# pyprob/pyprob

Hardware: NVIDIA H100
Metric: ic_train_traces_per_sec (higher is better)
Workload: dtype f32

## Files before the change

### pyprob_b200/csrc/net.cu

```cuda
#include <vector>
#include <string.h>
#include <stdlib.h>
#include <stdint.h>

#include "common.cuh"
#include "gemm_simt.cuh"
#include "heads.cuh"
#include "tc_grouped.cuh"
#include "tc_lstm.cuh"
#include "tc_cluster.cuh"
#include "tc_persist.cuh"
#include "obs_mlp.cuh"

using gemm::Problem;

struct HImg {
  float* k_hi = nullptr; float* k_lo = nullptr; float* mn_hi = nullptr; float* mn_lo = nullptr;
  int64_t kb = 0;
};

struct WImg {
  int64_t k_hi = 0, k_lo = 0, mn_hi = 0, mn_lo = 0;
  int kb = 0;
};
struct PackEntry {
  int64_t src_off;
  int rows, cols, ld, kb;
  int64_t k_hi, k_lo, mn_hi, mn_lo;
  int tile_start, pad_;
};

struct ppb_net {
  float* wimg = nullptr;
  int64_t wimg_floats = 0;
  std::vector<PackEntry> pack;
  PackEntry* d_pack = nullptr;
  int pack_tiles = 0;
  WImg w_ihE, w_hh;
  std::vector<WImg> w1, w2;
  WImg w_obs[PPB_MAX_OBS][PPB_MAX_FF_LAYERS];
  WImg w_fin[PPB_MAX_FF_LAYERS];
  int obs_tc = 0;
  uint64_t slot_hash[10] = {0, 0, 0, 0, 0, 0, 0, 0, 0, 0};
  const void* slot_dev[10] = {nullptr, nullptr, nullptr, nullptr, nullptr, nullptr, nullptr, nullptr, nullptr, nullptr};
  void* h_blob[2] = {nullptr, nullptr};
  cudaEvent_t ev_blob[2] = {nullptr, nullptr};
  size_t blob_cap = 0;
  int blob_idx = 0;
  ppb_net_desc desc;
  std::vector<ppb_addr_desc> addrs;
  std::vector<int64_t> type_off;
  ppb_addr_desc* d_addrs = nullptr;
  int64_t* d_type_off = nullptr;
  int64_t arena_floats = 0;
  int I = 0;
  int dh_pad = 4;
  int out_pad = 4;
  int fused_cell = 3;
  float* whh_il = nullptr;
  int64_t whh_il_floats = 0;
  void* d_lstm_steps = nullptr;
  size_t lstm_steps_cap = 0;
  int* d_lstm_progress = nullptr;
  int lstm_progress_cap = 0;
  int fused_cell_bwd = 1;
  void* d_bsteps = nullptr;
  size_t bsteps_cap = 0;
  cudaStream_t side[2] = {nullptr, nullptr};
  cudaEvent_t fork_ev[16] = {nullptr, nullptr, nullptr, nullptr, nullptr, nullptr, nullptr, nullptr,
                             nullptr, nullptr, nullptr, nullptr, nullptr, nullptr, nullptr, nullptr};
  int fork_next = 0;
  int single_stream = 0;
  int pack_tiles_no_hh = 0;
  int host_graph = 1;
  cudaStream_t host_stream = nullptr;
  cudaGraphExec_t host_exec = nullptr;
  uint64_t host_key = 0;
  int host_seen = 0;
  float* host_hyper_dev = nullptr;
  void* host_state_dev = nullptr;
  float host_hyper[6] = {0, 0, 0, 0, 0, 0};
  int64_t host_step_dev = -1;
  char* host_pin = nullptr;
  int64_t host_pin_cap = 0;
  Problem* h_stage[2] = {nullptr, nullptr};
  cudaEvent_t ev_stage[2] = {nullptr, nullptr};
  size_t stage_cap = 0;
  int stage_idx = 0;
};

namespace {

inline int64_t align_up(int64_t x, int64_t a) { return (x + a - 1) / a * a; }

struct Ws {
  float* obs_act[PPB_MAX_OBS][PPB_MAX_FF_LAYERS];
  float* obs_cat; float* fin_act[PPB_MAX_FF_LAYERS]; float* obs_emb;
  float* p_obs; float* emb_cat; float* p_step; float* w_smp_t; float* smp_emb;
  float* gates; float* c; float* h; float* hid; float* out_raw; float* row_lp; float* d_out;
  float* loss_acc;
  float* d_hid; float* dh; float* dh_rec; float* dc; float* d_pobs; float* d_pstep; float* d_smp; float* d_embcat;
  float* d_obs_emb; float* d_fin_act[PPB_MAX_FF_LAYERS]; float* d_obs_cat; float* d_obs_act[PPB_MAX_OBS][PPB_MAX_FF_LAYERS];
  Problem* problems;
  int64_t max_problems;
  int64_t total_bytes;
};

struct Dims {
  int B, R, T, NS, G;
};

Ws carve(const ppb_net* net, Dims d, void* base) {
  const ppb_net_desc& D = net->desc;
  Ws w;
  memset(&w, 0, sizeof(w));
  char* p = (char*)base;
  int64_t off = 0;
  auto take = [&](int64_t floats) {
    float* r = (float*)(p + off);
    off += align_up(floats * 4, 256);
    return r;
  };
  const int H = D.lstm_dim, E = D.obs_dim, S = D.sample_dim, C2 = 2 * (D.type_dim + D.addr_dim);
  for (int j = 0; j < D.num_obs; ++j)
    for (int l = 0; l + 1 < D.obs_ff[j].num_layers; ++l) w.obs_act[j][l] = take((int64_t)d.B * D.obs_ff[j].layers[l].out_dim);
  w.obs_cat = take((int64_t)d.B * E);
  for (int l = 0; l + 1 < D.obs_final.num_layers; ++l) w.fin_act[l] = take((int64_t)d.B * D.obs_final.layers[l].out_dim);
  w.obs_emb = take((int64_t)d.B * E);
  w.p_obs = take((int64_t)d.B * 4 * H);
  w.emb_cat = take((int64_t)d.NS * C2);
  w.p_step = take((int64_t)d.NS * 4 * H);
  w.w_smp_t = take((int64_t)S * 4 * H);
  w.smp_emb = take((int64_t)d.R * S);
  w.gates = take((int64_t)d.R * 4 * H);
  w.c = take((int64_t)d.R * H);
  w.h = take((int64_t)d.R * H);
  w.hid = take((int64_t)d.R * net->dh_pad);
  w.out_raw = take((int64_t)d.R * net->out_pad);
  w.row_lp = take(d.R);
  w.d_out = take((int64_t)d.R * net->out_pad);
  w.loss_acc = take(64);
  w.d_hid = take((int64_t)d.R * net->dh_pad);
  w.dh = take((int64_t)d.R * H);
  w.dh_rec = take((int64_t)d.R * H);
  w.dc = take((int64_t)d.R * H);
  w.d_pobs = take((int64_t)d.B * 4 * H);
  w.d_pstep = take((int64_t)d.NS * 4 * H);
  w.d_smp = take((int64_t)d.R * S);
  w.d_embcat = take((int64_t)d.NS * C2);
  w.d_obs_emb = take((int64_t)d.B * E);
  for (int l = 0; l + 1 < D.obs_final.num_layers; ++l) w.d_fin_act[l] = take((int64_t)d.B * D.obs_final.layers[l].out_dim);
  w.d_obs_cat = take((int64_t)d.B * E);
  for (int j = 0; j < D.num_obs; ++j)
    for (int l = 0; l + 1 < D.obs_ff[j].num_layers; ++l) w.d_obs_act[j][l] = take((int64_t)d.B * D.obs_ff[j].layers[l].out_dim);
  w.max_problems = 2 * (64 + 4LL * PPB_MAX_OBS * PPB_MAX_FF_LAYERS + 8LL * d.G + 4LL * d.T);
  w.problems = (Problem*)take(w.max_problems * (int64_t)(sizeof(Problem) / 4));
  w.total_bytes = off;
  return w;
}

inline float* dgates_ptr(const Ws& w, void* base) { return (float*)((char*)base + w.total_bytes); }
inline int64_t dgates_bytes(const ppb_net* net, Dims d) { return align_up((int64_t)d.R * 4 * net->desc.lstm_dim * 4, 256); }

struct Builder {
  std::vector<Problem> probs;
  std::vector<gemm::Phase> phases;
  void begin() { gemm::Phase ph; ph.first = (int)probs.size(); phases.push_back(ph); }
  void add(Problem p) {
    gemm::Phase& ph = phases.back();
    p.tiles_m = (p.M + gemm::BM - 1) / gemm::BM;
    p.tiles_n = (p.N + gemm::BN - 1) / gemm::BN;
    p.tile_start = ph.tiles;
    if (p.M <= 0 || p.N <= 0) return;
    ph.tiles += p.tiles_m * p.tiles_n;
    ph.count += 1;
    probs.push_back(p);
  }
};

inline Problem P0() {
  Problem p;
  memset(&p, 0, sizeof(p));
  p.alpha = 1.0f;
  return p;
}

inline Problem linear_fwd(const float* X, int64_t ldx, const float* W, int64_t ldw, const float* b, float* Y,
                          int64_t ldy, int M, int N, int K, int flags) {
  Problem p = P0();
  p.A = X; p.sam = ldx; p.sak = 1;
  p.B = W; p.sbn = ldw; p.sbk = 1;
  p.C = Y; p.ldc = ldy; p.bias = b;
  p.M = M; p.N = N; p.K = K; p.flags = flags;
  return p;
}
inline Problem linear_dx(const float* dY, int64_t lddy, const float* W, int64_t ldw, float* dX, int64_t lddx, int M,
                         int N, int K, int flags) {
  Problem p = P0();
  p.A = dY; p.sam = lddy; p.sak = 1;
  p.B = W; p.sbn = 1; p.sbk = ldw;
  p.C = dX; p.ldc = lddx;
  p.M = M; p.N = K; p.K = N; p.flags = flags;
  return p;
}
inline Problem linear_dw(const float* dY, int64_t lddy, const float* X, int64_t ldx, float* dW, int64_t ldw, int M,
                         int N, int K) {
  Problem p = P0();
  p.A = dY; p.sam = 1; p.sak = lddy;
  p.B = X; p.sbn = 1; p.sbk = ldx;
  p.C = dW; p.ldc = ldw;
  p.M = N; p.N = K; p.K = M; p.flags = gemm::kAccumulate;
  return p;
}

void add_obs_embed(Builder& bl, const ppb_net_desc& D, const float* arena, const float* obs, int B,
                   float* const (*obs_act)[PPB_MAX_FF_LAYERS], float* obs_cat, float* const* fin_act, float* obs_emb) {
  const int E = D.obs_dim;
  int max_depth = 0;
  for (int j = 0; j < D.num_obs; ++j) max_depth = D.obs_ff[j].num_layers > max_depth ? D.obs_ff[j].num_layers : max_depth;
  std::vector<int> in_off(D.num_obs), out_off(D.num_obs);
  { int ci = 0, co = 0; for (int j = 0; j < D.num_obs; ++j) { in_off[j] = ci; out_off[j] = co; ci += D.obs_ff[j].in_dim; co += D.obs_ff[j].out_dim; } }
  for (int l = 0; l < max_depth; ++l) {
    bl.begin();
    for (int j = 0; j < D.num_obs; ++j) {
      const ppb_ff_desc& ff = D.obs_ff[j];
      if (l >= ff.num_layers) continue;
      const ppb_linear_desc& L = ff.layers[l];
      const float* X = l == 0 ? obs + in_off[j] : obs_act[j][l - 1];
      int64_t ldx = l == 0 ? D.obs_in_total : ff.layers[l - 1].out_dim;
      bool last = (l == ff.num_layers - 1);
      float* Y = last ? obs_cat + out_off[j] : obs_act[j][l];
      int64_t ldy = last ? E : L.out_dim;
      bl.add(linear_fwd(X, ldx, arena + L.w_off, L.in_dim, arena + L.b_off, Y, ldy, B, L.out_dim, L.in_dim, gemm::kRelu));
    }
  }
  for (int l = 0; l < D.obs_final.num_layers; ++l) {
    bl.begin();
    const ppb_linear_desc& L = D.obs_final.layers[l];
    const float* X = l == 0 ? obs_cat : fin_act[l - 1];
    bool last = (l == D.obs_final.num_layers - 1);
    float* Y = last ? obs_emb : fin_act[l];
    bl.add(linear_fwd(X, L.in_dim, arena + L.w_off, L.in_dim, arena + L.b_off, Y, L.out_dim, B, L.out_dim, L.in_dim, gemm::kRelu));
  }
}

inline uint64_t fnv1a(const void* data, size_t n, uint64_t h = 1469598103934665603ULL) {
  const unsigned char* p = (const unsigned char*)data;
  for (size_t i = 0; i < n; ++i) { h ^= p[i]; h *= 1099511628211ULL; }
  return h;
}

int upload_cached(ppb_net* net, int slot, const void* src, size_t bytes, void* dev, cudaStream_t st) {
  if (bytes == 0) return PPB_OK;
  uint64_t h = fnv1a(src, bytes, 1469598103934665603ULL ^ (uint64_t)bytes);
  if (net->slot_hash[slot] == h && net->slot_dev[slot] == dev) return PPB_OK;
  cudaStreamCaptureStatus cap = cudaStreamCaptureStatusNone;
  cudaStreamIsCapturing(st, &cap);
  if (cap != cudaStreamCaptureStatusNone) {
    ppb_set_error("the batch structure changed inside a CUDA-graph capture: run the step once eagerly first");
    return PPB_EINVAL;
  }
  if (net->blob_cap < bytes) {
    for (int i = 0; i < 2; ++i) {
      if (net->h_blob[i]) cudaFreeHost(net->h_blob[i]);
      PPB_CUDA(cudaMallocHost(&net->h_blob[i], bytes * 2));
      if (!net->ev_blob[i]) PPB_CUDA(cudaEventCreateWithFlags(&net->ev_blob[i], cudaEventDisableTiming));
    }
    net->blob_cap = bytes * 2;
  }
  int i = net->blob_idx;
  net->blob_idx ^= 1;
  PPB_CUDA(cudaEventSynchronize(net->ev_blob[i]));
  memcpy(net->h_blob[i], src, bytes);
  PPB_CUDA(cudaMemcpyAsync(dev, net->h_blob[i], bytes, cudaMemcpyHostToDevice, st));
  PPB_CUDA(cudaEventRecord(net->ev_blob[i], st));
  net->slot_hash[slot] = h;
  net->slot_dev[slot] = dev;
  return PPB_OK;
}

int upload_and_get(ppb_net* net, const Builder& b, Problem* dev, int64_t cap, cudaStream_t st, int slot = 0) {
  size_t n = b.probs.size();
  if ((int64_t)n > cap) { ppb_set_error("problem list overflow (%zu > %lld)", n, (long long)cap); return PPB_ENOMEM; }
  return upload_cached(net, slot, b.probs.data(), n * sizeof(Problem), dev, st);
}

int stream_after(ppb_net* net, cudaStream_t from, cudaStream_t to) {
  if (from == to) return PPB_OK;
  cudaEvent_t& ev = net->fork_ev[net->fork_next];
  net->fork_next = (net->fork_next + 1) & 15;
  if (!ev) PPB_CUDA(cudaEventCreateWithFlags(&ev, cudaEventDisableTiming));
  PPB_CUDA(cudaEventRecord(ev, from));
  PPB_CUDA(cudaStreamWaitEvent(to, ev, 0));
  return PPB_OK;
}
int side_stream(ppb_net* net, int k, cudaStream_t main_st, cudaStream_t* out) {
  if (net->single_stream) { *out = main_st; return PPB_OK; }
  if (!net->side[k]) PPB_CUDA(cudaStreamCreateWithFlags(&net->side[k], cudaStreamNonBlocking));
  *out = net->side[k];
  return PPB_OK;
}

struct Prof {
  bool on = false;
  std::vector<std::pair<cudaEvent_t, cudaEvent_t>> spans;
  double flops = 0.0;
  int64_t launches = 0;
} g_prof;

int run_phase(const gemm::Phase& ph, const Problem* dev, cudaStream_t st, const Builder* bl_for_prof = nullptr) {
  if (ph.count == 0) return PPB_OK;
  int grid = ph.tiles < 8 * PPB_NUM_SMS ? ph.tiles : 8 * PPB_NUM_SMS;
  cudaEvent_t e0 = nullptr, e1 = nullptr;
  const bool prof = g_prof.on && bl_for_prof;
  if (prof) {
    PPB_CUDA(cudaEventCreate(&e0));
    PPB_CUDA(cudaEventCreate(&e1));
    PPB_CUDA(cudaEventRecord(e0, st));
  }
  gemm::k_grouped<<<grid, gemm::kThreads, 0, st>>>(dev + ph.first, ph.count, ph.tiles);
  PPB_LAUNCH_CHECK();
  if (prof) {
    PPB_CUDA(cudaEventRecord(e1, st));
    g_prof.spans.push_back({e0, e1});
    g_prof.launches += 1;
    for (int i = 0; i < ph.count; ++i) {
      const Problem& p = bl_for_prof->probs[ph.first + i];
      g_prof.flops += 2.0 * p.M * p.N * p.K;
    }
  }
  return PPB_OK;
}

__global__ void k_step_embed(const float* __restrict__ arena, const ppb_addr_desc* __restrict__ addrs,
                             const int64_t* __restrict__ type_off, const int* __restrict__ step_addr,
                             const int* __restrict__ step_prev, int n_steps, int td, int ad,
                             float* __restrict__ emb_cat) {
  int C2 = 2 * (td + ad);
  for (int64_t e = (int64_t)blockIdx.x * blockDim.x + threadIdx.x; e < (int64_t)n_steps * C2;
       e += (int64_t)gridDim.x * blockDim.x) {
    int st = (int)(e / C2), j = (int)(e % C2);
    int which = j < (td + ad) ? step_prev[st] : step_addr[st];
    int jj = j < (td + ad) ? j : j - (td + ad);
    float v = 0.0f;
    if (which >= 0) {
      const ppb_addr_desc& a = addrs[which];
      v = jj < td ? arena[type_off[a.type_id] + jj] : arena[a.addr_emb_off + (jj - td)];
    }
    emb_cat[e] = v;
  }
}

__global__ void k_wsmp_transpose(const float* __restrict__ w_ih, int I, int E, int S, int H4,
                                 float* __restrict__ w_smp_t) {
  for (int e = blockIdx.x * blockDim.x + threadIdx.x; e < S * H4; e += gridDim.x * blockDim.x) {
    int j = e / H4, col = e % H4;
    w_smp_t[e] = w_ih[(int64_t)col * I + E + j];
  }
}

__global__ void k_smp_embed(const float* __restrict__ arena, const ppb_addr_desc* __restrict__ addrs,
                            const int* __restrict__ row_step, const int* __restrict__ step_prev,
                            const int* __restrict__ row_prev, const float* __restrict__ values, int R, int S,
                            float* __restrict__ smp_emb) {
  for (int64_t e = (int64_t)blockIdx.x * blockDim.x + threadIdx.x; e < (int64_t)R * S;
       e += (int64_t)gridDim.x * blockDim.x) {
    int row = (int)(e / S), j = (int)(e % S);
    int pa = step_prev[row_step[row]];
    float v = 0.0f;
    if (pa >= 0) {
      const ppb_addr_desc& a = addrs[pa];
      float x = values[row_prev[row]];
      const float* W = arena + a.smp_w_off + (int64_t)j * a.smp_in;
      float pre = arena[a.smp_b_off + j];
      if (a.family == PPB_FAMILY_CATEGORICAL) {
        int c = (int)x;
        if (c >= 0 && c < a.smp_in) pre += W[c];
      } else {
        pre += W[0] * x;
      }
      v = fmaxf(pre, 0.0f);
    }
    smp_emb[e] = v;
  }
}

__global__ void __launch_bounds__(256) k_cell_fwd(float* __restrict__ gates, const float* __restrict__ p_obs,
                                                   const float* __restrict__ p_step, const float* __restrict__ w_smp_t,
                                                   const float* __restrict__ smp_emb, const int* __restrict__ row_step,
                                                   const int* __restrict__ row_prev, const int* __restrict__ row_trace,
                                                   float* __restrict__ c, float* __restrict__ h, HImg himg, int row0,
                                                   int n_rows, int H, int S, int t) {
  ppb_pdl_trigger();
  ppb_pdl_wait();
  int64_t total = (int64_t)n_rows * H;
  for (int64_t e = (int64_t)blockIdx.x * blockDim.x + threadIdx.x; e < total; e += (int64_t)gridDim.x * blockDim.x) {
    int i = (int)(e / H), j = (int)(e % H);
    int row = row0 + i;
    int st = row_step[row];
    int tr = row_trace[row];
    if (tr < 0) {
      gates[(int64_t)row * 4 * H + j] = 0.f; gates[(int64_t)row * 4 * H + H + j] = 0.f;
      gates[(int64_t)row * 4 * H + 2 * H + j] = 0.f; gates[(int64_t)row * 4 * H + 3 * H + j] = 0.f;
      c[(int64_t)row * H + j] = 0.f; h[(int64_t)row * H + j] = 0.f;
      if (himg.k_hi) tcg::img_store(himg.k_hi, himg.k_lo, himg.mn_hi, himg.mn_lo, row, j, himg.kb, 0.0f);
      continue;
    }
    float pre[4];
#pragma unroll
    for (int g = 0; g < 4; ++g) {
      int col = g * H + j;
      float v = p_obs[(int64_t)tr * 4 * H + col] + p_step[(int64_t)st * 4 * H + col];
      if (t > 0) {
        v += gates[(int64_t)row * 4 * H + col];
        for (int s = 0; s < S; ++s) v = fmaf(smp_emb[(int64_t)row * S + s], w_smp_t[(int64_t)s * 4 * H + col], v);
      }
      pre[g] = v;
    }
    float ig = ppb_cell_sigmoid(pre[0]);
    float fg = ppb_cell_sigmoid(pre[1]);
    float gg = ppb_cell_tanh(pre[2]);
    float og = ppb_cell_sigmoid(pre[3]);
    float cp = (t > 0) ? c[(int64_t)row_prev[row] * H + j] : 0.0f;
    float cn = fg * cp + ig * gg;
    float hn = og * ppb_cell_tanh(cn);
    gates[(int64_t)row * 4 * H + j] = ig;
    gates[(int64_t)row * 4 * H + H + j] = fg;
    gates[(int64_t)row * 4 * H + 2 * H + j] = gg;
    gates[(int64_t)row * 4 * H + 3 * H + j] = og;
    c[(int64_t)row * H + j] = cn;
    h[(int64_t)row * H + j] = hn;
    if (himg.k_hi) tcg::img_store(himg.k_hi, himg.k_lo, himg.mn_hi, himg.mn_lo, row, j, himg.kb, hn);
  }
}

struct NllArgs {
  const ppb_addr_desc* addrs;
  const int* row_step; const int* step_addr;
  const float* values; const float* prior0; const float* prior1;
  const int* row_trace;
  int K; float inv_batch;
  float* row_lp; float* d_out; int out_pad;
  HImg dimg;
};
__device__ __forceinline__ void nll_row(const NllArgs& A, const float* x, int row, int lane, float& local, int& bad) {
  const ppb_addr_desc* addrs = A.addrs;
  const int* row_step = A.row_step; const int* step_addr = A.step_addr;
  const float* values = A.values; const float* prior0 = A.prior0; const float* prior1 = A.prior1;
  const int* row_trace = A.row_trace;
  const int K = A.K, out_pad = A.out_pad;
  const float inv_batch = A.inv_batch;
  float* row_lp = A.row_lp; float* d_out = A.d_out;
// ... 1592 lines not shown
```

### pyprob_b200/csrc/net_tc.inc

```
extern unsigned long long* g_trace;
extern int g_trace_launch;

namespace {

inline int64_t img_floats(int64_t rows, int64_t cols) {
  return ((rows + 127) / 128) * ((cols + 31) / 32) * tc::kTileFloats;
}

__global__ void __launch_bounds__(256) k_pack_table(const float* __restrict__ arena, const PackEntry* __restrict__ tab,
                                                     int n_entries, float* __restrict__ wimg) {
  int tile = blockIdx.x;
  int lo = 0, hi = n_entries - 1;
  while (lo < hi) {
    int mid = (lo + hi + 1) >> 1;
    if (tab[mid].tile_start <= tile) lo = mid; else hi = mid - 1;
  }
  const PackEntry e = tab[lo];
  const int rt = tile - e.tile_start;
  const float* src = arena + e.src_off;
  for (int q = threadIdx.x + blockIdx.y * blockDim.x; q < 128 * e.kb * 8; q += blockDim.x * gridDim.y) {
    int c16 = q & 7, t = q >> 3;
    int cb = t % e.kb, r = t / e.kb;
    int row = rt * 128 + r, k0 = cb * 32 + c16 * 4;
    float h[4], l[4];
// ... 116 lines not shown
  net->w1.clear();
  net->w2.clear();
  for (auto& a : net->addrs) {
    net->w1.push_back(add(a.w1_off, a.head_hidden, H, H));
    net->w2.push_back(add(a.w2_off, a.head_out, a.head_hidden, a.head_hidden));
  }
  net->obs_tc = obs_tc_ok(D) ? 1 : 0;
  if (net->obs_tc) {
    for (int j = 0; j < D.num_obs; ++j)
      for (int l = 1; l < D.obs_ff[j].num_layers; ++l) {
        const ppb_linear_desc& L = D.obs_ff[j].layers[l];
        net->w_obs[j][l] = add(L.w_off, L.out_dim, L.in_dim, L.in_dim);
      }
    for (int l = 0; l < D.obs_final.num_layers; ++l) {
      const ppb_linear_desc& L = D.obs_final.layers[l];
      net->w_fin[l] = add(L.w_off, L.out_dim, L.in_dim, L.in_dim);
    }
  }
  net->pack_tiles_no_hh = tiles;
  net->w_hh = add(D.w_hh_off, 4 * H, H, H);
  net->pack_tiles = tiles;
  if (net->wimg) cudaFree(net->wimg);
  if (net->d_pack) cudaFree(net->d_pack);
  net->wimg_floats = off;
  PPB_CUDA(cudaMalloc((void**)&net->wimg, off * sizeof(float)));
  PPB_CUDA(cudaMalloc((void**)&net->d_pack, net->pack.size() * sizeof(PackEntry)));
  PPB_CUDA(cudaMemcpy(net->d_pack, net->pack.data(), net->pack.size() * sizeof(PackEntry), cudaMemcpyHostToDevice));
  if (net->fused_cell) {
    if (net->whh_il) cudaFree(net->whh_il);
    net->whh_il_floats = img_floats(4 * H, H);
    PPB_CUDA(cudaMalloc((void**)&net->whh_il, 2 * net->whh_il_floats * sizeof(float)));
  }
  return PPB_OK;
}

struct LstmPhase { int first = 0, count = 0, tiles = 0; };

template <bool X3>
int launch_lstm_seq(int tiles, const tcl::Seq* dev, int n, cudaStream_t st) {
  static bool attr_set = false;
  if (!attr_set) {
    PPB_CUDA(cudaFuncSetAttribute(tcl::k_lstm_seq<X3>, cudaFuncAttributeMaxDynamicSharedMemorySize, (int)tcl::smem_bytes()));
    attr_set = true;
  }
  tcl::k_lstm_seq<X3><<<tiles, tcg::kThreads, tcl::smem_bytes(), st>>>(dev, n);
  return PPB_OK;
}

template <bool X3>
int launch_lstm_step(const LstmPhase& ph, const tcl::Step* dev, cudaStream_t st) {
  static bool attr_set = false;
  if (!attr_set) {
    PPB_CUDA(cudaFuncSetAttribute(tcl::k_lstm_step<X3>, cudaFuncAttributeMaxDynamicSharedMemorySize, (int)tcl::smem_bytes()));
    attr_set = true;
  }
  tcl::k_lstm_step<X3><<<ph.tiles, tcg::kThreads, tcl::smem_bytes(), st>>>(dev + ph.first, ph.count);
  return PPB_OK;
}

struct TcWs {
  HImg obs_emb, h, hid, d_out, d_hid, dgates, dpobs;
  HImg a_img[PPB_MAX_OBS][PPB_MAX_FF_LAYERS], cat_img, fin_img[PPB_MAX_FF_LAYERS];
  HImg g_act[PPB_MAX_OBS][PPB_MAX_FF_LAYERS], g_cat, g_fin[PPB_MAX_FF_LAYERS], g_emb;
  char* obs_img_begin; int64_t obs_img_bytes;
  tcg::Problem* probs;
  int* ints;
  int64_t max_probs, max_ints;
  int64_t total_bytes;
};

TcWs carve_tc(const ppb_net* net, Dims d, void* base) {
  const ppb_net_desc& D = net->desc;
  TcWs w;
  char* p = (char*)base;
  int64_t off = 0;
  auto take = [&](int64_t floats) { float* r = (float*)(p + off); off += align_up(floats * 4, 1024); return r; };
  auto img = [&](int64_t rows, int64_t cols) {
    HImg im;
    int64_t n = img_floats(rows, cols);
    im.kb = (cols + 31) / 32;
    im.k_hi = take(n); im.k_lo = take(n); im.mn_hi = take(n); im.mn_lo = take(n);
    return im;
  };
  const int H = D.lstm_dim;
  w.obs_emb = img(d.B, D.obs_dim);
  w.h = img(d.R, H);
  w.hid = img(d.R, net->dh_pad);
  w.d_out = img(d.R, net->out_pad);
  w.d_hid = img(d.R, net->dh_pad);
  w.dgates = img(d.R, 4 * H);
  w.dpobs = img(d.B, 4 * H);
  w.obs_img_begin = p + off;
  if (net->obs_tc) {
    for (int j = 0; j < D.num_obs; ++j)
      for (int l = 0; l + 1 < D.obs_ff[j].num_layers; ++l) {
        w.a_img[j][l] = img(d.B, D.obs_ff[j].layers[l].out_dim);
        w.g_act[j][l] = img(d.B, D.obs_ff[j].layers[l].out_dim);
      }
    w.cat_img = img(d.B, D.obs_dim);
    w.g_cat = img(d.B, D.obs_dim);
    for (int l = 0; l + 1 < D.obs_final.num_layers; ++l) {
      w.fin_img[l] = img(d.B, D.obs_final.layers[l].out_dim);
      w.g_fin[l] = img(d.B, D.obs_final.layers[l].out_dim);
    }
    w.g_emb = img(d.B, D.obs_dim);
  }
  w.obs_img_bytes = (p + off) - w.obs_img_begin;
  w.max_probs = 2 * (16 + 6LL * d.NS + 4LL * d.G + 4LL * (PPB_MAX_OBS * PPB_MAX_FF_LAYERS + PPB_MAX_FF_LAYERS));
  w.probs = (tcg::Problem*)take(w.max_probs * (int64_t)(sizeof(tcg::Problem) / 4));
  w.max_ints = 64 + 4LL * (d.R / 32 + d.NS);
  w.ints = (int*)take(w.max_ints);
  w.total_bytes = off;
  return w;
}

inline int64_t simt_region_bytes(const ppb_net* net, Dims d) {
  return align_up(carve(net, d, nullptr).total_bytes + dgates_bytes(net, d), 1024);
}

struct TcBuilder {
  std::vector<tcg::Problem> probs;
  std::vector<gemm::Phase> phases;
  std::vector<int> ints;
  void begin() { gemm::Phase ph; ph.first = (int)probs.size(); phases.push_back(ph); }
  void add(tcg::Problem p) {
    gemm::Phase& ph = phases.back();
    if (p.M <= 0 || p.N <= 0 || p.K <= 0) return;
    p.tiles_m = (p.M + 127) / 128;
    p.tiles_n = (p.N + 127) / 128;
    p.tile_start = ph.tiles;
    if (p.k_splits < 1) p.k_splits = 1;
    ph.tiles += p.tiles_m * p.tiles_n * p.k_splits;
    ph.count += 1;
    probs.push_back(p);
  }
};

inline tcg::Operand op_k(const float* hi, const float* lo, int kb, int row0, int col0) {
  tcg::Operand o; o.hi = hi; o.lo = lo; o.k_rows = nullptr; o.kb = kb; o.mn = 0; o.row0 = row0; o.col0 = col0; return o;
}
inline tcg::Operand op_mn(const float* hi, const float* lo, int kb, int row0, int col0, const int* k_rows = nullptr) {
  tcg::Operand o; o.hi = hi; o.lo = lo; o.k_rows = k_rows; o.kb = kb; o.mn = 1; o.row0 = row0; o.col0 = col0; return o;
}
inline tcg::Problem TP0() { tcg::Problem p; memset(&p, 0, sizeof(p)); return p; }
inline tcg::Operand wk(const ppb_net* net, const WImg& w) { return op_k(net->wimg + w.k_hi, net->wimg + w.k_lo, w.kb, 0, 0); }
inline tcg::Operand wmn(const ppb_net* net, const WImg& w) { return op_mn(net->wimg + w.mn_hi, net->wimg + w.mn_lo, w.kb, 0, 0); }

inline bool tc_persistent_on() {
  const char* e = getenv("PPB_PERSISTENT");
  return !(e && e[0] == '0');
}

template <bool X3, int EPI>
int launch_tc(const gemm::Phase& ph, const tcg::Problem* dev, cudaStream_t st, unsigned long long* tr) {
  static bool attr_set = false;
  if (!attr_set) {
    PPB_CUDA(cudaFuncSetAttribute(tcg::k_grouped<X3, EPI>, cudaFuncAttributeMaxDynamicSharedMemorySize, (int)tcg::smem_bytes()));
    attr_set = true;
  }
  if (tc_persistent_on() && ph.tiles > PPB_NUM_SMS && tr == nullptr) {
    static bool attr_p = false;
    if (!attr_p) {
      PPB_CUDA(cudaFuncSetAttribute(tcp::k_grouped_persistent<X3, EPI>, cudaFuncAttributeMaxDynamicSharedMemorySize,
                                    (int)tcp::smem_bytes()));
      attr_p = true;
    }
    PPB_CUDA(ppb_launch(tcp::k_grouped_persistent<X3, EPI>, dim3(PPB_NUM_SMS), dim3(tcg::kThreads), tcp::smem_bytes(), st, 1, 0,
                        dev + ph.first, ph.count, ph.tiles));
    return PPB_OK;
  }
  PPB_CUDA(ppb_launch(tcg::k_grouped<X3, EPI>, dim3((unsigned)ph.tiles), dim3(tcg::kThreads), tcg::smem_bytes(), st, 1, 0,
                      dev + ph.first, ph.count, tr));
  return PPB_OK;
}

int run_tc_phase(const gemm::Phase& ph, const tcg::Problem* dev, int precision, cudaStream_t st, int epi,
                 const TcBuilder* bl_for_prof = nullptr) {
  if (ph.count == 0) return PPB_OK;
  cudaEvent_t e0 = nullptr, e1 = nullptr;
  const bool prof = g_prof.on && bl_for_prof;
  if (prof) {
    PPB_CUDA(cudaEventCreate(&e0));
    PPB_CUDA(cudaEventCreate(&e1));
    PPB_CUDA(cudaEventRecord(e0, st));
  }
  unsigned long long* tr = nullptr;
  if (g_trace && g_trace_launch < 256) { tr = g_trace + 16 * g_trace_launch; ++g_trace_launch; }
  int rc2 = PPB_OK;
  const bool x3 = precision == PPB_PREC_TF32X3;
  if (epi == 0) rc2 = x3 ? launch_tc<true, 0>(ph, dev, st, tr) : launch_tc<false, 0>(ph, dev, st, tr);
  else if (epi == 1) rc2 = x3 ? launch_tc<true, 1>(ph, dev, st, tr) : launch_tc<false, 1>(ph, dev, st, tr);
  else rc2 = x3 ? launch_tc<true, 2>(ph, dev, st, tr) : launch_tc<false, 2>(ph, dev, st, tr);
  if (rc2) return rc2;
  PPB_LAUNCH_CHECK();
  if (prof) {
    PPB_CUDA(cudaEventRecord(e1, st));
    g_prof.spans.push_back({e0, e1});
    g_prof.launches += 1;
    for (int i = 0; i < ph.count; ++i) {
      const tcg::Problem& p = bl_for_prof->probs[ph.first + i];
      g_prof.flops += 2.0 * p.M * p.N * p.K;
    }
  }
  return PPB_OK;
}

inline int pick_cluster(int tiles, int min_kc, bool spread_epilogue = false) {
  static const bool off = [] { const char* e = getenv("PPB_NO_CLUSTER"); return e && e[0] == '1'; }();
  if (off) return 1;
  int cs = 1;
  while (cs < 8 && tiles * cs * 2 <= PPB_NUM_SMS && (spread_epilogue || min_kc / (cs * 2) >= 2)) cs *= 2;
  return cs;
}

template <bool X3, int CS, int EPI>
int launch_cluster_tc(const gemm::Phase& ph, const tcg::Problem* dev, cudaStream_t st) {
  static bool attr_set = false;
  if (!attr_set) {
    PPB_CUDA(cudaFuncSetAttribute(tcc::k_cluster<X3, CS, EPI>, cudaFuncAttributeMaxDynamicSharedMemorySize, (int)tcc::smem_bytes()));
    attr_set = true;
  }
  unsigned long long* tr = nullptr;
  if (g_trace && g_trace_launch < 256) { tr = g_trace + 16 * g_trace_launch; ++g_trace_launch; }
  PPB_CUDA(tcc::launch_cluster(tcc::k_cluster<X3, CS, EPI>, ph.tiles * CS, CS, tcc::smem_bytes(), st, dev + ph.first, ph.count, tr));
  return PPB_OK;
}
template <bool X3, int EPI>
int launch_cluster_cs(int cs, const gemm::Phase& ph, const tcg::Problem* dev, cudaStream_t st) {
  if (cs == 2) return launch_cluster_tc<X3, 2, EPI>(ph, dev, st);
  if (cs == 4) return launch_cluster_tc<X3, 4, EPI>(ph, dev, st);
  return launch_cluster_tc<X3, 8, EPI>(ph, dev, st);
}

int run_tc_phase_auto(const gemm::Phase& ph, const tcg::Problem* dev, int precision, cudaStream_t st, int epi,
                      const TcBuilder& tb, bool profile = false) {
  if (ph.count == 0) return PPB_OK;
  int min_kc = 1 << 30;
  for (int i = 0; i < ph.count; ++i) {
    const tcg::Problem& p = tb.probs[ph.first + i];
    if (p.k_splits > 1) return run_tc_phase(ph, dev, precision, st, epi, profile ? &tb : nullptr);
    int kc = (p.K + 31) / 32;
    min_kc = kc < min_kc ? kc : min_kc;
  }
  static const bool spread = [] { const char* e = getenv("PPB_SPREAD_EPILOGUE"); return !(e && e[0] == '0'); }();
  const int cs = pick_cluster(ph.tiles, min_kc, epi == 2 && spread);
  if (cs == 1 || (epi != 0 && epi != 2)) return run_tc_phase(ph, dev, precision, st, epi, profile ? &tb : nullptr);
  cudaEvent_t e0 = nullptr, e1 = nullptr;
  const bool prof = g_prof.on && profile;
  if (prof) {
    PPB_CUDA(cudaEventCreate(&e0));
    PPB_CUDA(cudaEventCreate(&e1));
    PPB_CUDA(cudaEventRecord(e0, st));
  }
  const bool x3 = precision == PPB_PREC_TF32X3;
  int rc2;
  if (epi == 0) rc2 = x3 ? launch_cluster_cs<true, 0>(cs, ph, dev, st) : launch_cluster_cs<false, 0>(cs, ph, dev, st);
  else rc2 = x3 ? launch_cluster_cs<true, 2>(cs, ph, dev, st) : launch_cluster_cs<false, 2>(cs, ph, dev, st);
  if (rc2) return rc2;
  PPB_LAUNCH_CHECK();
  if (prof) {
    PPB_CUDA(cudaEventRecord(e1, st));
    g_prof.spans.push_back({e0, e1});
    g_prof.launches += 1;
    for (int i = 0; i < ph.count; ++i) {
      const tcg::Problem& p = tb.probs[ph.first + i];
      g_prof.flops += 2.0 * p.M * p.N * p.K;
    }
  }
  return PPB_OK;
}

template <bool X3, int CS, int SMAX>
int launch_lstm_cluster_s(const LstmPhase& ph, const tcl::Step* dev, cudaStream_t st) {
  static bool attr_set = false;
  if (!attr_set) {
    PPB_CUDA(cudaFuncSetAttribute(tcc::k_lstm_cluster<X3, CS, SMAX>, cudaFuncAttributeMaxDynamicSharedMemorySize,
                                  (int)tcc::smem_bytes()));
    attr_set = true;
  }
  unsigned long long* tr = nullptr;
  if (g_trace && g_trace_launch < 256) { tr = g_trace + 16 * g_trace_launch; ++g_trace_launch; }
  PPB_CUDA(tcc::launch_cluster(tcc::k_lstm_cluster<X3, CS, SMAX>, ph.tiles * CS, CS, tcc::smem_bytes(), st, dev + ph.first,
                               ph.count, tr));
  return PPB_OK;
}
template <bool X3, int CS>
int launch_lstm_cluster(const LstmPhase& ph, const tcl::Step* dev, int S, cudaStream_t st) {
  return S <= 4 ? launch_lstm_cluster_s<X3, CS, 4>(ph, dev, st) : launch_lstm_cluster_s<X3, CS, 8>(ph, dev, st);
}

template <bool X3, int CS>
int launch_lstm_bwd_cluster(const LstmPhase& ph, const tcc::BStep* dev, cudaStream_t st) {
  static bool attr_set = false;
  if (!attr_set) {
    PPB_CUDA(cudaFuncSetAttribute(tcc::k_lstm_bwd_cluster<X3, CS>, cudaFuncAttributeMaxDynamicSharedMemorySize, (int)tcc::smem_bytes()));
    attr_set = true;
  }
  PPB_CUDA(tcc::launch_cluster(tcc::k_lstm_bwd_cluster<X3, CS>, ph.tiles * CS, CS, tcc::smem_bytes(), st, dev + ph.first, ph.count));
  return PPB_OK;
}

inline int pad128(int n) { return (n + 127) / 128 * 128; }

inline obsmlp::Net obs_net_of(const ppb_net_desc& D) {
  obsmlp::Net n;
  n.num_obs = D.num_obs; n.obs_in_total = D.obs_in_total; n.E = D.obs_dim;
  for (int j = 0; j < PPB_MAX_OBS; ++j) n.obs_ff[j] = D.obs_ff[j];
  n.obs_final = D.obs_final;
  return n;
}
inline bool obs_fused_ok(const ppb_net_desc& D, int B) {
  constexpr int kFuseMaxWidth = obsmlp::W2;
  if (D.obs_dim > kFuseMaxWidth) return false;
  for (int j = 0; j < D.num_obs; ++j)
    for (int l = 0; l < D.obs_ff[j].num_layers; ++l)
      if (D.obs_ff[j].layers[l].in_dim > kFuseMaxWidth || D.obs_ff[j].layers[l].out_dim > kFuseMaxWidth) return false;
  for (int l = 0; l < D.obs_final.num_layers; ++l)
    if (D.obs_final.layers[l].in_dim > kFuseMaxWidth || D.obs_final.layers[l].out_dim > kFuseMaxWidth) return false;
  (void)B;
  return obsmlp::smem_bytes2(obs_net_of(D)) <= 200 * 1024;
}
inline obsmlp::Bufs obs_bufs_of(const Ws& w) {
  obsmlp::Bufs b;
  for (int j = 0; j < PPB_MAX_OBS; ++j)
    for (int l = 0; l < PPB_MAX_FF_LAYERS; ++l) b.obs_act[j][l] = w.obs_act[j][l];
  b.obs_cat = w.obs_cat;
  for (int l = 0; l < PPB_MAX_FF_LAYERS; ++l) b.fin_act[l] = w.fin_act[l];
  b.obs_emb = w.obs_emb;
  return b;
}
inline obsmlp::DBufs obs_dbufs_of(const Ws& w) {
  obsmlp::DBufs b;
  for (int j = 0; j < PPB_MAX_OBS; ++j)
    for (int l = 0; l < PPB_MAX_FF_LAYERS; ++l) b.d_obs_act[j][l] = w.d_obs_act[j][l];
  b.d_obs_cat = w.d_obs_cat;
  for (int l = 0; l < PPB_MAX_FF_LAYERS; ++l) b.d_fin_act[l] = w.d_fin_act[l];
  b.d_obs_emb = w.d_obs_emb;
  return b;
}
inline int obs_traces_per_cta(int B) {
  int t = (B + PPB_NUM_SMS - 1) / PPB_NUM_SMS;
  t = (t + obsmlp::kWarps - 1) / obsmlp::kWarps * obsmlp::kWarps;
  return t < obsmlp::kWarps ? obsmlp::kWarps : t;
}
int obs_fused_fwd(const ppb_net_desc& D, const float* arena, const float* obs, int B, const Ws& w, cudaStream_t st,
                  const HImg* emb_img = nullptr) {
  static bool attr = false;
  if (!attr) {
    PPB_CUDA(cudaFuncSetAttribute(obsmlp::k_fwd2, cudaFuncAttributeMaxDynamicSharedMemorySize, 200 * 1024));
    PPB_CUDA(cudaFuncSetAttribute(obsmlp::k_bwd2_dx, cudaFuncAttributeMaxDynamicSharedMemorySize, 200 * 1024));
    attr = true;
  }
  const obsmlp::Net n = obs_net_of(D);
  const int tpc = obs_traces_per_cta(B);
  obsmlp::Bufs bufs = obs_bufs_of(w);
  if (emb_img) {
    bufs.emb_k_hi = emb_img->k_hi; bufs.emb_k_lo = emb_img->k_lo; bufs.emb_mn_hi = emb_img->mn_hi; bufs.emb_mn_lo = emb_img->mn_lo;
    bufs.emb_kb = emb_img->kb;
  }
  obsmlp::k_fwd2<<<(B + tpc - 1) / tpc, obsmlp::kWarps * 32, obsmlp::smem_bytes2(n), st>>>(n, arena, obs, B, tpc, bufs);
  PPB_LAUNCH_CHECK();
  return PPB_OK;
}
int obs_fused_bwd(const ppb_net_desc& D, const float* arena, float* grad, const float* obs, int B, const Ws& w,
                  cudaStream_t st) {
  const obsmlp::Net n = obs_net_of(D);
  const int tpc = obs_traces_per_cta(B);
  PPB_CUDA(ppb_launch(obsmlp::k_bwd2_dx, dim3((B + tpc - 1) / tpc), dim3(obsmlp::kWarps * 32), obsmlp::smem_bytes2(n), st, 2,
                      0, n, arena, B, tpc, obs_bufs_of(w), obs_dbufs_of(w)));
  PPB_LAUNCH_CHECK();
  obsmlp::DwTable tab;
  memset(&tab, 0, sizeof(tab));
  int total = 0;
  auto add = [&](const float* dy, int ldy, const float* x, int ldx, const ppb_linear_desc& L) {
    obsmlp::DwLayer& e = tab.layer[tab.n_layers++];
    e.dy = dy; e.ldy = ldy; e.x = x; e.ldx = ldx; e.out_dim = L.out_dim; e.in_dim = L.in_dim;
    e.w_off = L.w_off; e.b_off = L.b_off; e.start = total;
    total += L.out_dim * L.in_dim + L.out_dim;
  };
  const int E = D.obs_dim;
  for (int l = 0; l < D.obs_final.num_layers; ++l) {
    const ppb_linear_desc& L = D.obs_final.layers[l];
    const bool last = l == D.obs_final.num_layers - 1;
    add(last ? w.d_obs_emb : w.d_fin_act[l], L.out_dim, l == 0 ? w.obs_cat : w.fin_act[l - 1], L.in_dim, L);
  }
  int in_off = 0, out_off = 0;
  for (int j = 0; j < D.num_obs; ++j) {
    const ppb_ff_desc& ff = D.obs_ff[j];
    for (int l = 0; l < ff.num_layers; ++l) {
      const ppb_linear_desc& L = ff.layers[l];
      const bool last = l == ff.num_layers - 1;
      const float* dy = last ? w.d_obs_cat + out_off : w.d_obs_act[j][l];
      const float* x = l == 0 ? obs + in_off : w.obs_act[j][l - 1];
      add(dy, last ? E : L.out_dim, x, l == 0 ? D.obs_in_total : ff.layers[l - 1].out_dim, L);
    }
    in_off += ff.in_dim;
    out_off += ff.out_dim;
  }
  tab.total = total;
  const int b_chunk = 512;
  PPB_CUDA(ppb_launch(obsmlp::k_dw, dim3((total + 31) / 32, (B + b_chunk - 1) / b_chunk), dim3(256), 0, st, 2, 0, tab, B,
                      b_chunk, grad));
  PPB_LAUNCH_CHECK();
  return PPB_OK;
}

inline int pick_splits(int M, int N, int K, int phase_tiles = 0) {
  int tiles = ((M + 127) / 128) * ((N + 127) / 128), kc = (K + 31) / 32;
  if (phase_tiles > tiles) tiles = phase_tiles;
  int s = PPB_NUM_SMS / tiles;
  if (s > kc / 2) s = kc / 2;
  return s < 1 ? 1 : s;
}

__global__ void __launch_bounds__(256) k_head_bias_grad(const float* __restrict__ d_out, int out_pad,
                                                         const float* __restrict__ d_hid, int dh_pad,
                                                         const int* __restrict__ head_rows, const int* __restrict__ group_start,
                                                         const int* __restrict__ group_addr,
                                                         const ppb_addr_desc* __restrict__ addrs, float* __restrict__ grad) {
  __shared__ float part[8][33];
  const int g = blockIdx.y;
  const ppb_addr_desc a = addrs[group_addr[g]];
  const int hid_blocks = (dh_pad + 31) / 32;
  const bool is_hid = (int)blockIdx.x < hid_blocks;
  const int lane = threadIdx.x & 31, slice = threadIdx.x >> 5;
  const int n = (is_hid ? blockIdx.x : blockIdx.x - hid_blocks) * 32 + lane;
  const int width = is_hid ? a.head_hidden : a.head_out;
  const float* src = is_hid ? d_hid : d_out;
  const int ld = is_hid ? dh_pad : out_pad;
  const int s0 = group_start[g], cnt = group_start[g + 1] - s0;
  float s = 0.0f;
  if (n < width)
    for (int m = slice; m < cnt; m += 8) s += src[(int64_t)head_rows[s0 + m] * ld + n];
  part[slice][lane] = s;
  __syncthreads();
  if (slice == 0 && n < width) {
    float t = 0.0f;
#pragma unroll
    for (int k = 0; k < 8; ++k) t += part[k][lane];
    if (t != 0.0f) atomicAdd(grad + (is_hid ? a.b1_off : a.b2_off) + n, t);
  }
}

__global__ void __launch_bounds__(256) k_pstep_fwd(const float* __restrict__ emb_cat, const float* __restrict__ w_ih,
                                                    const float* __restrict__ b_ih, const float* __restrict__ b_hh,
                                                    int NS, int H4, int I, int off, int C2, float* __restrict__ p_step) {
  int warp = (blockIdx.x * blockDim.x + threadIdx.x) >> 5, lane = threadIdx.x & 31;
  int nw = (gridDim.x * blockDim.x) >> 5;
  for (int o = warp; o < NS * H4; o += nw) {
    int st = o / H4, col = o % H4;
    float s = 0.0f;
    for (int j = lane; j < C2; j += 32) s = fmaf(emb_cat[(int64_t)st * C2 + j], w_ih[(int64_t)col * I + off + j], s);
    s = ppb_warp_sum(s);
    if (lane == 0) p_step[o] = s + b_ih[col] + b_hh[col];
  }
}
__global__ void __launch_bounds__(256) k_pstep_dx(const float* __restrict__ d_pstep, const float* __restrict__ w_ih,
                                                   int H4, int I, int off, int C2, float* __restrict__ d_embcat) {
  __shared__ float part[8][33];
  const int st = blockIdx.y, lane = threadIdx.x & 31, slice = threadIdx.x >> 5;
  const int j = blockIdx.x * 32 + lane;
  float s = 0.0f;
  if (j < C2)
    for (int col = blockIdx.z * 8 + slice; col < H4; col += 8 * gridDim.z)
      s = fmaf(d_pstep[(int64_t)st * H4 + col], w_ih[(int64_t)col * I + off + j], s);
  part[slice][lane] = s;
  __syncthreads();
  if (slice == 0 && j < C2) {
    float t = 0.0f;
#pragma unroll
    for (int k = 0; k < 8; ++k) t += part[k][lane];
    atomicAdd(d_embcat + (int64_t)st * C2 + j, t);
  }
}
__global__ void __launch_bounds__(256) k_pstep_dw(const float* __restrict__ d_pstep, const float* __restrict__ emb_cat,
                                                   int NS, int H4, int I, int off, int C2, float* __restrict__ dw_ih) {
  for (int64_t e = (int64_t)blockIdx.x * blockDim.x + threadIdx.x; e < (int64_t)H4 * C2;
       e += (int64_t)gridDim.x * blockDim.x) {
    int col = (int)(e / C2), j = (int)(e % C2);
    float s = 0.0f;
    for (int st = 0; st < NS; ++st) s = fmaf(d_pstep[(int64_t)st * H4 + col], emb_cat[(int64_t)st * C2 + j], s);
    dw_ih[(int64_t)col * I + off + j] += s;
  }
}

int check_tc(const ppb_net* net, const ppb_batch* b) {
  PPB_CHECK_ARG(b->row_align == 128, "the tensor-core path needs a batch encoded with row_align = 128");
  PPB_CHECK_ARG(net->wimg != nullptr, "weight images not built (ppb_net_set_tables)");
  PPB_CHECK_ARG(net->desc.lstm_dim % 32 == 0, "tensor-core path: lstm_dim must be a multiple of 32");
  PPB_CHECK_ARG(b->step_addr_host && b->step_row0_host && b->step_nrows_host && b->step_t_host && b->step_prev_row0_host,
                "missing per-step host arrays");
  return PPB_OK;
}

int tc_loss_forward(ppb_net* net, const float* arena, const ppb_batch* b, void* workspace, int precision,
                    float* loss_out, int32_t* status_out, float* row_lp_out, int want_grad, cudaStream_t st) {
  int rc = check_tc(net, b);
  if (rc) return rc;
  const ppb_net_desc& D = net->desc;
  Dims d = dims_of(b);
  Ws w = carve(net, d, workspace);
  TcWs t = carve_tc(net, d, (char*)workspace + simt_region_bytes(net, d));
  const int H = D.lstm_dim, H4 = 4 * H, E = D.obs_dim, S = D.sample_dim, I = net->I;
  const int C2 = 2 * (D.type_dim + D.addr_dim);
  const int dhkb = (net->dh_pad + 31) / 32;

  Builder bl;
  const bool fused_obs = obs_fused_ok(D, d.B);
  const bool obs_tc = !fused_obs && net->obs_tc;
  std::vector<int> obs_in_off(D.num_obs), obs_out_off(D.num_obs);
  { int ci = 0, co = 0; for (int j = 0; j < D.num_obs; ++j) { obs_in_off[j] = ci; obs_out_off[j] = co; ci += D.obs_ff[j].in_dim; co += D.obs_ff[j].out_dim; } }
  if (obs_tc) {
    bl.begin();
    for (int j = 0; j < D.num_obs; ++j) {
      const ppb_linear_desc& L = D.obs_ff[j].layers[0];
      bl.add(linear_fwd(b->obs + obs_in_off[j], D.obs_in_total, arena + L.w_off, L.in_dim, arena + L.b_off, w.obs_act[j][0],
                        L.out_dim, d.B, L.out_dim, L.in_dim, gemm::kRelu));
    }
  } else if (!fused_obs) {
    add_obs_embed(bl, D, arena, b->obs, d.B, w.obs_act, w.obs_cat, w.fin_act, w.obs_emb);
  }
  const int ph_pstep = (int)bl.phases.size();
  rc = upload_and_get(net, bl, w.problems, w.max_problems / 2, st, 0);
  if (rc) return rc;

  TcBuilder tb;
  std::vector<int> ph_obs_tc;
  if (obs_tc) {
    auto set_out = [](tcg::Problem& p, const HImg& im, int col0) {
      p.o_k_hi = im.k_hi; p.o_k_lo = im.k_lo; p.o_mn_hi = im.mn_hi; p.o_mn_lo = im.mn_lo;
      p.o_kb = (int)im.kb; p.o_row0 = 0; p.o_col0 = col0;
    };
    int max_depth = 0;
    for (int j = 0; j < D.num_obs; ++j) max_depth = D.obs_ff[j].num_layers > max_depth ? D.obs_ff[j].num_layers : max_depth;
    for (int l = 1; l < max_depth; ++l) {
      ph_obs_tc.push_back((int)tb.phases.size());
      tb.begin();
      for (int j = 0; j < D.num_obs; ++j) {
        const ppb_ff_desc& ff = D.obs_ff[j];
        if (l >= ff.num_layers) continue;
        const ppb_linear_desc& L = ff.layers[l];
        const bool last = l == ff.num_layers - 1;
        tcg::Problem p = TP0();
        p.a = op_k(t.a_img[j][l - 1].k_hi, t.a_img[j][l - 1].k_lo, (int)t.a_img[j][l - 1].kb, 0, 0);
        p.b = wk(net, net->w_obs[j][l]);
        p.M = d.B; p.N = L.out_dim; p.K = L.in_dim;
        p.flags = tcg::kRelu; p.bias = arena + L.b_off;
        if (last) { set_out(p, t.cat_img, obs_out_off[j]); p.c = w.obs_cat + obs_out_off[j]; p.ldc = E; }
        else { set_out(p, t.a_img[j][l], 0); p.c = w.obs_act[j][l]; p.ldc = L.out_dim; }
        tb.add(p);
      }
    }
    for (int l = 0; l < D.obs_final.num_layers; ++l) {
      const ppb_linear_desc& L = D.obs_final.layers[l];
      const bool last = l == D.obs_final.num_layers - 1;
      const HImg& in = l == 0 ? t.cat_img : t.fin_img[l - 1];
      ph_obs_tc.push_back((int)tb.phases.size());
      tb.begin();
      tcg::Problem p = TP0();
      p.a = op_k(in.k_hi, in.k_lo, (int)in.kb, 0, 0);
      p.b = wk(net, net->w_fin[l]);
      p.M = d.B; p.N = L.out_dim; p.K = L.in_dim;
      p.flags = tcg::kRelu; p.bias = arena + L.b_off;
      if (last) { set_out(p, t.obs_emb, 0); p.c = w.obs_emb; p.ldc = L.out_dim; }
      else { set_out(p, t.fin_img[l], 0); p.c = w.fin_act[l]; p.ldc = L.out_dim; }
      tb.add(p);
    }
  }
  const int ph_pobs = (int)tb.phases.size();
  tb.begin();
  {
    tcg::Problem p = TP0();
    p.a = op_k(t.obs_emb.k_hi, t.obs_emb.k_lo, (int)t.obs_emb.kb, 0, 0);
    p.b = wk(net, net->w_ihE);
    p.M = d.B; p.N = H4; p.K = E;
    p.c = w.p_obs; p.ldc = H4;
    tb.add(p);
  }
  std::vector<int> ph_rec(d.T, -1);
  {
    int st0 = 0;
    for (int tt = 0; tt < d.T; ++tt) {
      int st1 = st0;
      while (st1 < d.NS && b->step_t_host[st1] == tt) ++st1;
      if (tt > 0) {
        ph_rec[tt] = (int)tb.phases.size();
        tb.begin();
        for (int s = st0; s < st1; ++s) {
          tcg::Problem p = TP0();
          p.a = op_k(t.h.k_hi, t.h.k_lo, (int)t.h.kb, b->step_prev_row0_host[s], 0);
          p.b = wk(net, net->w_hh);
          p.M = pad128(b->step_nrows_host[s]); p.N = H4; p.K = H;
          p.c = w.gates + (int64_t)b->step_row0_host[s] * H4; p.ldc = H4;
          tb.add(p);
        }
      }
      st0 = st1;
    }
  }
  const int ph_h1 = (int)tb.phases.size();
  tb.begin();
  for (int s = 0; s < d.NS; ++s) {
    int aid = b->step_addr_host[s];
    const ppb_addr_desc& a = net->addrs[aid];
    tcg::Problem p = TP0();
    p.a = op_k(t.h.k_hi, t.h.k_lo, (int)t.h.kb, b->step_row0_host[s], 0);
    p.b = wk(net, net->w1[aid]);
    p.M = pad128(b->step_nrows_host[s]); p.N = a.head_hidden; p.K = H;
    p.m_valid = b->step_nrows_host[s];
    p.flags = tcg::kRelu | tcg::kZeroInvalid;
    p.bias = arena + a.b1_off;
    p.o_k_hi = t.hid.k_hi; p.o_k_lo = t.hid.k_lo; p.o_mn_hi = t.hid.mn_hi; p.o_mn_lo = t.hid.mn_lo;
    p.o_kb = dhkb; p.o_row0 = b->step_row0_host[s]; p.o_col0 = 0;
    tb.add(p);
  }
  const int ph_h2 = (int)tb.phases.size();
  tb.begin();
  for (int s = 0; s < d.NS; ++s) {
    int aid = b->step_addr_host[s];
    const ppb_addr_desc& a = net->addrs[aid];
    tcg::Problem p = TP0();
    p.a = op_k(t.hid.k_hi, t.hid.k_lo, dhkb, b->step_row0_host[s], 0);
    p.b = wk(net, net->w2[aid]);
    p.M = pad128(b->step_nrows_host[s]); p.N = a.head_out; p.K = a.head_hidden;
    p.bias = arena + a.b2_off;
    p.c = w.out_raw + (int64_t)b->step_row0_host[s] * net->out_pad; p.ldc = net->out_pad;
    tb.add(p);
  }
  PPB_CHECK_ARG((int64_t)tb.probs.size() <= t.max_probs / 2, "tensor-core problem list overflow");
  rc = upload_cached(net, 2, tb.probs.data(), tb.probs.size() * sizeof(tcg::Problem), t.probs, st);
  if (rc) return rc;

  std::vector<tcl::Step> lsteps;
  std::vector<LstmPhase> lphase(d.T);
  const bool fused_cell = net->fused_cell && net->whh_il && d.T > 1;
  bool persistent = false;
  int seq_tiles = 0, seq_count = 0, seq_counters = 0;
  if (fused_cell) {
    tcl::CellIO io;
    memset(&io, 0, sizeof(io));
    io.p_obs = w.p_obs; io.p_step = w.p_step; io.smp_emb = w.smp_emb; io.w_smp_t = w.w_smp_t;
    io.row_trace = b->row_trace; io.row_step = b->row_step; io.row_prev = b->row_prev;
    io.gates = w.gates; io.c = w.c; io.h = w.h;
    io.hk_hi = t.h.k_hi; io.hk_lo = t.h.k_lo; io.hmn_hi = t.h.mn_hi; io.hmn_lo = t.h.mn_lo; io.hkb = (int)t.h.kb;
    { static const bool nb = [] { const char* e = getenv("PPB_LSTM_B_PREFETCH"); return e && e[0] == '0'; }(); io.no_b_prefetch = nb ? 1 : 0; }
    io.H = H; io.S = S;
    const tcg::Operand a_img = op_k(t.h.k_hi, t.h.k_lo, (int)t.h.kb, 0, 0);
    const tcg::Operand b_img = op_k(net->whh_il, net->whh_il + net->whh_il_floats, H / 32, 0, 0);
    std::vector<int> seg_first(d.T + 1, 0);
    {
      int st0 = 0;
      for (int tt = 0; tt < d.T; ++tt) {
        int st1 = st0;
        while (st1 < d.NS && b->step_t_host[st1] == tt) ++st1;
        seg_first[tt] = st0;
        seg_first[tt + 1] = st1;
        st0 = st1;
      }
    }
    const int n_sub1 = seg_first[2] - seg_first[1];
    std::vector<tcl::Seq> seqs;
    if (net->fused_cell == 2) {
      for (int j = 0; j < n_sub1; ++j) {
        const int s1 = seg_first[1] + j;
        tcl::Seq q;
        memset(&q, 0, sizeof(q));
        q.a = a_img; q.b = b_img;
        q.M = pad128(b->step_nrows_host[s1]);
        q.T = 1;
        for (int tt = 1; tt < d.T; ++tt)
          if (seg_first[tt + 1] - seg_first[tt] > j) q.T = tt + 1;
        q.seg_off = b->step_row0_host[s1] - b->row_off_host[1];
        q.tiles_m = q.M / 128; q.tiles_n = H / 32;
        q.tile_start = seq_tiles;
        q.prog0 = seq_counters;
        seq_tiles += q.tiles_m * q.tiles_n;
        seq_counters += q.tiles_m;
        q.io = io;
        seqs.push_back(q);
      }
      seq_count = (int)seqs.size();
      persistent = seq_count > 0 && seq_tiles <= PPB_NUM_SMS;
    }
    size_t bytes = 0;
    std::vector<char> blob;
    if (persistent) {
      const size_t seq_bytes = seqs.size() * sizeof(tcl::Seq);
      bytes = seq_bytes + (size_t)(d.T + 1) * sizeof(int);
      blob.resize(bytes);
    } else {
      for (int tt = 1; tt < d.T; ++tt) {
        lphase[tt].first = (int)lsteps.size();
        for (int s = seg_first[tt]; s < seg_first[tt + 1]; ++s) {
          tcl::Step q;
          memset(&q, 0, sizeof(q));
          q.a = a_img; q.a.row0 = b->step_prev_row0_host[s];
          q.b = b_img;
          q.M = pad128(b->step_nrows_host[s]);
          q.row0 = b->step_row0_host[s];
          q.tiles_m = q.M / 128; q.tiles_n = H / 32;
          q.tile_start = lphase[tt].tiles;
          lphase[tt].tiles += q.tiles_m * q.tiles_n;
          lphase[tt].count += 1;
          q.io = io;
          lsteps.push_back(q);
        }
      }
      bytes = lsteps.size() * sizeof(tcl::Step);
    }
    cudaStreamCaptureStatus cap = cudaStreamCaptureStatusNone;
    cudaStreamIsCapturing(st, &cap);
    if (net->lstm_steps_cap < bytes) {
      PPB_CHECK_ARG(cap == cudaStreamCaptureStatusNone, "fused LSTM step list must be built once outside a graph capture");
      if (net->d_lstm_steps) cudaFree(net->d_lstm_steps);
      PPB_CUDA(cudaMalloc(&net->d_lstm_steps, bytes * 2));
      net->lstm_steps_cap = bytes * 2;
      net->slot_hash[7] = 0;
    }
    if (persistent) {
      if (net->lstm_progress_cap < seq_counters + 1) {
        PPB_CHECK_ARG(cap == cudaStreamCaptureStatusNone, "fused LSTM counters must be allocated outside a graph capture");
        if (net->d_lstm_progress) cudaFree(net->d_lstm_progress);
        PPB_CUDA(cudaMalloc((void**)&net->d_lstm_progress, (size_t)(seq_counters + 1) * 2 * sizeof(int)));
        net->lstm_progress_cap = (seq_counters + 1) * 2;
      }
      const size_t seq_bytes = seqs.size() * sizeof(tcl::Seq);
      for (auto& q : seqs) {
        q.row_off = (const int*)((const char*)net->d_lstm_steps + seq_bytes);
        q.progress = net->d_lstm_progress;
        q.n_counters = seq_counters;
      }
      memcpy(blob.data(), seqs.data(), seq_bytes);
      memcpy(blob.data() + seq_bytes, b->row_off_host, (size_t)(d.T + 1) * sizeof(int));
      rc = upload_cached(net, 7, blob.data(), bytes, net->d_lstm_steps, st);
    } else {
      rc = upload_cached(net, 7, lsteps.data(), bytes, net->d_lstm_steps, st);
    }
    if (rc) return rc;
  }

  cudaStream_t s1, s2;
  rc = side_stream(net, 0, st, &s1); if (rc) return rc;
  rc = side_stream(net, 1, st, &s2); if (rc) return rc;
  rc = stream_after(net, st, s1); if (rc) return rc;
  rc = stream_after(net, st, s2); if (rc) return rc;
  PPB_CUDA(cudaMemsetAsync(w.loss_acc, 0, 256, s1));
  k_pack_table<<<dim3(d.T > 1 ? net->pack_tiles : net->pack_tiles_no_hh, 8), 256, 0, s2>>>(arena, net->d_pack,
                                                                                         (int)net->pack.size(), net->wimg);
  PPB_LAUNCH_CHECK();
  if (fused_cell) {
    tcl::k_pack_whh_interleaved<<<dim3(H / 32, 8), 256, 0, s2>>>(arena + D.w_hh_off, H, net->whh_il,
                                                                 net->whh_il + net->whh_il_floats);
    PPB_LAUNCH_CHECK();
  }
  k_step_embed<<<ew_grid((int64_t)d.NS * C2), 256, 0, s1>>>(arena, net->d_addrs, net->d_type_off, b->step_addr,
                                                            b->step_prev_addr, d.NS, D.type_dim, D.addr_dim, w.emb_cat);
  PPB_LAUNCH_CHECK();
  k_pstep_fwd<<<ew_grid((int64_t)d.NS * H4 * 32), 256, 0, s1>>>(w.emb_cat, arena + D.w_ih_off, arena + D.b_ih_off,
                                                                arena + D.b_hh_off, d.NS, H4, I, E + S, C2, w.p_step);
  PPB_LAUNCH_CHECK();
  if (d.T > 1) {
    k_wsmp_transpose<<<ew_grid(S * H4), 256, 0, s1>>>(arena + D.w_ih_off, I, E, S, H4, w.w_smp_t);
    PPB_LAUNCH_CHECK();
    k_smp_embed<<<ew_grid((int64_t)d.R * S), 256, 0, s1>>>(arena, net->d_addrs, b->row_step, b->step_prev_addr,
                                                           b->row_prev, b->values, d.R, S, w.smp_emb);
    PPB_LAUNCH_CHECK();
  }
  static const bool emb_fuse_on = [] { const char* e = getenv("PPB_FUSE_PACK"); return !(e && e[0] == '0'); }();
  const bool emb_packed = fused_obs && emb_fuse_on && (d.B & 127) == 0 && (E & 31) == 0;
  if (fused_obs) { rc = obs_fused_fwd(D, arena, b->obs, d.B, w, st, emb_packed ? &t.obs_emb : nullptr); if (rc) return rc; }
  if (obs_tc && (d.B & 127))
    PPB_CUDA(cudaMemsetAsync(t.obs_img_begin, 0, (size_t)t.obs_img_bytes, st));
  for (int l = 0; l < ph_pstep; ++l) { rc = run_phase(bl.phases[l], w.problems, st); if (rc) return rc; }
  if (obs_tc) {
    for (int j = 0; j < D.num_obs; ++j) {
      const int od = D.obs_ff[j].layers[0].out_dim;
      PPB_CUDA(ppb_launch(k_pack_rows, dim3(dim3((d.B + 127) / 128, 4)), dim3(256), 0, st, 1, 0, w.obs_act[j][0], d.B, od, od, t.a_img[j][0]));
      PPB_LAUNCH_CHECK();
    }
    rc = stream_after(net, s2, st); if (rc) return rc;
    for (int ph : ph_obs_tc) { rc = run_tc_phase_auto(tb.phases[ph], t.probs, precision, st, 2, tb); if (rc) return rc; }
  } else {
    if (!emb_packed) {
      PPB_CUDA(ppb_launch(k_pack_rows, dim3(dim3((d.B + 127) / 128, 4)), dim3(256), 0, st, 1, 0, w.obs_emb, d.B, E, E, t.obs_emb));
      PPB_LAUNCH_CHECK();
// ... 138 lines not shown
    const ppb_addr_desc& a = net->addrs[aid];
    tcg::Problem p = TP0();
    p.a = op_k(t.d_out.k_hi, t.d_out.k_lo, okb, b->step_row0_host[s], 0);
    p.b = wmn(net, net->w2[aid]);
    p.M = pad128(b->step_nrows_host[s]); p.N = a.head_hidden; p.K = a.head_out;
    p.flags = tcg::kMaskImg;
    p.mask_hi = t.hid.k_hi;
    p.c = w.d_hid + (int64_t)b->step_row0_host[s] * net->dh_pad; p.ldc = net->dh_pad;
    p.o_k_hi = t.d_hid.k_hi; p.o_k_lo = t.d_hid.k_lo; p.o_mn_hi = t.d_hid.mn_hi; p.o_mn_lo = t.d_hid.mn_lo;
    p.o_kb = dhkb; p.o_row0 = b->step_row0_host[s]; p.o_col0 = 0;
    tb.add(p);
  }
  const int ph_hw = (int)tb.phases.size();
  tb.begin();
  for (int s = 0; s < d.NS; ++s) {
    int aid = b->step_addr_host[s];
    const ppb_addr_desc& a = net->addrs[aid];
    tcg::Problem p = TP0();
    p.a = op_k(t.d_hid.k_hi, t.d_hid.k_lo, dhkb, b->step_row0_host[s], 0);
    p.b = wmn(net, net->w1[aid]);
    p.M = pad128(b->step_nrows_host[s]); p.N = H; p.K = a.head_hidden;
    p.c = w.dh + (int64_t)b->step_row0_host[s] * H; p.ldc = H;
    tb.add(p);
  }
  const int ph_headw = (int)tb.phases.size();
  tb.begin();
  int headw_tiles = 0;
  for (size_t aid = 0; aid < net->addrs.size(); ++aid) {
    if (chunk_off[aid] < 0) continue;
    const ppb_addr_desc& a = net->addrs[aid];
    headw_tiles += ((a.head_out + 127) / 128) * ((a.head_hidden + 127) / 128) + ((a.head_hidden + 127) / 128) * ((H + 127) / 128);
  }
  for (size_t aid = 0; aid < net->addrs.size(); ++aid) {
    if (chunk_off[aid] < 0) continue;
    const ppb_addr_desc& a = net->addrs[aid];
    const int* kr = t.ints + chunk_off[aid];
    int nch = (int)addr_chunks[aid].size();
    tcg::Problem p2 = TP0();
    p2.a = op_mn(t.d_out.mn_hi, t.d_out.mn_lo, okb, 0, 0, kr);
    p2.b = op_mn(t.hid.mn_hi, t.hid.mn_lo, dhkb, 0, 0, kr);
    p2.M = a.head_out; p2.N = a.head_hidden; p2.K = 32 * nch;
    p2.c = grad + a.w2_off; p2.ldc = a.head_hidden; p2.flags = tcg::kAccumulate;
    p2.k_splits = pick_splits(p2.M, p2.N, p2.K, headw_tiles);
    tb.add(p2);
    tcg::Problem p1 = TP0();
    p1.a = op_mn(t.d_hid.mn_hi, t.d_hid.mn_lo, dhkb, 0, 0, kr);
    p1.b = op_mn(t.h.mn_hi, t.h.mn_lo, hkb, 0, 0, kr);
    p1.M = a.head_hidden; p1.N = H; p1.K = 32 * nch;
    p1.c = grad + a.w1_off; p1.ldc = H; p1.flags = tcg::kAccumulate;
    p1.k_splits = pick_splits(p1.M, p1.N, p1.K, headw_tiles);
    tb.add(p1);
  }
  std::vector<int> ph_rec(d.T, -1);
  std::vector<char> rec_cluster(d.T, 0);
  {
    int st1 = d.NS;
    for (int tt = d.T - 1; tt >= 1; --tt) {
      int st0 = st1;
      while (st0 > 0 && b->step_t_host[st0 - 1] == tt) --st0;
      ph_rec[tt] = (int)tb.phases.size();
      tb.begin();
      for (int s = st0; s < st1; ++s) {
        tcg::Problem p = TP0();
        p.a = op_k(t.dgates.k_hi, t.dgates.k_lo, gkb, b->step_row0_host[s], 0);
        p.b = wmn(net, net->w_hh);
        p.M = pad128(b->step_nrows_host[s]); p.N = H; p.K = H4;
        p.c = w.dh_rec + (int64_t)b->step_prev_row0_host[s] * H; p.ldc = H;
        tb.add(p);
      }
      {
        gemm::Phase& ph = tb.phases.back();
        static const int dx_cluster = [] { const char* e = getenv("PPB_REC_DX_CLUSTER"); return (e && e[0] >= '1' && e[0] <= '8') ? e[0] - '0' : 0; }();
        rec_cluster[tt] = dx_cluster && pick_cluster(ph.tiles, H4 / 32) > 1;
        if (!rec_cluster[tt]) {
          int rows = 0;
          for (int i = 0; i < ph.count; ++i) rows += tb.probs[ph.first + i].M;
          const int splits = pick_splits(rows, H, H4);
          ph.tiles = 0;
          for (int i = 0; i < ph.count; ++i) {
            tcg::Problem& p = tb.probs[ph.first + i];
            p.k_splits = splits;
            p.tile_start = ph.tiles;
            ph.tiles += p.tiles_m * p.tiles_n * splits;
          }
        }
      }
      st1 = st0;
    }
  }
  std::vector<tcc::BStep> bsteps;
  std::vector<LstmPhase> bphase(d.T);
  std::vector<int> bcs(d.T, 0);
  if (net->fused_cell_bwd) {
    tcc::BwdIO io;
    memset(&io, 0, sizeof(io));
    io.gates = w.gates; io.c = w.c; io.dh = w.dh; io.dc = w.dc; io.dgates = dgates; io.d_pobs = w.d_pobs;
    io.row_prev = b->row_prev; io.row_next = b->row_next; io.row_trace = b->row_trace;
    io.gk_hi = t.dgates.k_hi; io.gk_lo = t.dgates.k_lo; io.gmn_hi = t.dgates.mn_hi; io.gmn_lo = t.dgates.mn_lo;
    io.gkb = gkb; io.H = H;
    for (int tt = d.T - 1; tt >= 1; --tt) {
      if (!rec_cluster[tt]) continue;
      const gemm::Phase& ph = tb.phases[ph_rec[tt]];
      bcs[tt] = pick_cluster(ph.tiles, H4 / 32);
      {
        static const int cap = [] { const char* e = getenv("PPB_REC_DX_CLUSTER"); return (e && e[0] >= '2' && e[0] <= '8') ? e[0] - '0' : 8; }();
        while (bcs[tt] > cap) bcs[tt] >>= 1;
      }
      bphase[tt].first = (int)bsteps.size();
      for (int i = 0; i < ph.count; ++i) {
        const tcg::Problem& p = tb.probs[ph.first + i];
        tcc::BStep q;
        memset(&q, 0, sizeof(q));
        q.a = p.a; q.b = p.b; q.M = p.M;
        q.row0 = (int)((p.c - w.dh_rec) / H);
        q.t = tt - 1;
        q.tiles_m = p.tiles_m; q.tiles_n = p.tiles_n;
        q.tile_start = bphase[tt].tiles;
        bphase[tt].tiles += q.tiles_m * q.tiles_n;
        bphase[tt].count += 1;
        q.io = io;
        bsteps.push_back(q);
      }
    }
    const size_t bytes = bsteps.size() * sizeof(tcc::BStep);
    if (bytes > 0) {
      if (net->bsteps_cap < bytes) {
        cudaStreamCaptureStatus cap = cudaStreamCaptureStatusNone;
        cudaStreamIsCapturing(st, &cap);
        PPB_CHECK_ARG(cap == cudaStreamCaptureStatusNone, "fused BPTT step list must be built once outside a graph capture");
        if (net->d_bsteps) cudaFree(net->d_bsteps);
        PPB_CUDA(cudaMalloc(&net->d_bsteps, bytes * 2));
        net->bsteps_cap = bytes * 2;
        net->slot_hash[8] = 0;
      }
      rc = upload_cached(net, 8, bsteps.data(), bytes, net->d_bsteps, st);
      if (rc) return rc;
    }
  }

  const int ph_lstm_w = (int)tb.phases.size();
  tb.begin();
  if (!hh_a.empty()) {
    tcg::Problem p = TP0();
    p.a = op_mn(t.dgates.mn_hi, t.dgates.mn_lo, gkb, 0, 0, t.ints + hh_a_off);
    p.b = op_mn(t.h.mn_hi, t.h.mn_lo, hkb, 0, 0, t.ints + hh_b_off);
    p.M = H4; p.N = H; p.K = 32 * (int)hh_a.size();
    p.c = grad + D.w_hh_off; p.ldc = H; p.flags = tcg::kAccumulate;
    p.k_splits = pick_splits(p.M, p.N, p.K);
    tb.add(p);
  }
  {
    tcg::Problem p = TP0();
    p.a = op_mn(t.dpobs.mn_hi, t.dpobs.mn_lo, gkb, 0, 0);
    p.b = op_mn(t.obs_emb.mn_hi, t.obs_emb.mn_lo, (int)t.obs_emb.kb, 0, 0);
    p.M = H4; p.N = E; p.K = pad128(d.B);
    p.c = grad + D.w_ih_off; p.ldc = I; p.flags = tcg::kAccumulate;
    p.k_splits = pick_splits(p.M, p.N, p.K);
    tb.add(p);
    tcg::Problem q = TP0();
    q.a = op_k(t.dpobs.k_hi, t.dpobs.k_lo, gkb, 0, 0);
    q.b = wmn(net, net->w_ihE);
    q.M = d.B; q.N = E; q.K = H4;
    q.c = w.d_obs_emb; q.ldc = E;
    q.k_splits = pick_splits(q.M, q.N, q.K);
    tb.add(q);
  }
  const bool fused_obs = obs_fused_ok(D, d.B);
  const bool obs_tc = !fused_obs && net->obs_tc;
  std::vector<int> ph_bobs_dx;
  int ph_bobs_dw = -1;
  std::vector<int> obs_in_off(D.num_obs), obs_out_off(D.num_obs);
  { int ci = 0, co = 0; for (int j = 0; j < D.num_obs; ++j) { obs_in_off[j] = ci; obs_out_off[j] = co; ci += D.obs_ff[j].in_dim; co += D.obs_ff[j].out_dim; } }
  int obs_max_depth = 0;
  for (int j = 0; j < D.num_obs; ++j) obs_max_depth = D.obs_ff[j].num_layers > obs_max_depth ? D.obs_ff[j].num_layers : obs_max_depth;
  if (obs_tc) {
    const int Bp = pad128(d.B);
    auto set_out = [](tcg::Problem& p, const HImg& im) {
      p.o_k_hi = im.k_hi; p.o_k_lo = im.k_lo; p.o_mn_hi = im.mn_hi; p.o_mn_lo = im.mn_lo;
      p.o_kb = (int)im.kb; p.o_row0 = 0; p.o_col0 = 0;
    };
    struct DwSpec { const HImg* gy; int gy_col0; const HImg* x; const ppb_linear_desc* L; };
    std::vector<DwSpec> dws;
    for (int l = D.obs_final.num_layers - 1; l >= 0; --l) {
      const ppb_linear_desc& L = D.obs_final.layers[l];
      const HImg& gy = (l == D.obs_final.num_layers - 1) ? t.g_emb : t.g_fin[l];
      const HImg& x = l == 0 ? t.cat_img : t.fin_img[l - 1];
      const HImg& gx = l == 0 ? t.g_cat : t.g_fin[l - 1];
      ph_bobs_dx.push_back((int)tb.phases.size());
      tb.begin();
      tcg::Problem p = TP0();
      p.a = op_k(gy.k_hi, gy.k_lo, (int)gy.kb, 0, 0);
      p.b = wmn(net, net->w_fin[l]);
      p.M = d.B; p.N = L.in_dim; p.K = L.out_dim;
      p.flags = tcg::kMaskImg; p.mask_hi = x.k_hi;
      p.c = l == 0 ? w.d_obs_cat : w.d_fin_act[l - 1]; p.ldc = L.in_dim;
      set_out(p, gx);
      tb.add(p);
      dws.push_back({&gy, 0, &x, &L});
    }
    for (int l = obs_max_depth - 1; l >= 1; --l) {
      ph_bobs_dx.push_back((int)tb.phases.size());
      tb.begin();
      for (int j = 0; j < D.num_obs; ++j) {
        const ppb_ff_desc& ff = D.obs_ff[j];
        if (l >= ff.num_layers) continue;
        const ppb_linear_desc& L = ff.layers[l];
        const bool last = l == ff.num_layers - 1;
        const HImg& gy = last ? t.g_cat : t.g_act[j][l];
        const int gy_col0 = last ? obs_out_off[j] : 0;
        const HImg& x = t.a_img[j][l - 1];
        tcg::Problem p = TP0();
        p.a = op_k(gy.k_hi, gy.k_lo, (int)gy.kb, 0, gy_col0);
        p.b = wmn(net, net->w_obs[j][l]);
        p.M = d.B; p.N = L.in_dim; p.K = L.out_dim;
        p.flags = tcg::kMaskImg; p.mask_hi = x.k_hi;
        p.c = w.d_obs_act[j][l - 1]; p.ldc = L.in_dim;
        set_out(p, t.g_act[j][l - 1]);
        tb.add(p);
        dws.push_back({&gy, gy_col0, &x, &L});
      }
    }
    ph_bobs_dw = (int)tb.phases.size();
    tb.begin();
    int dw_tiles = 0;
    for (auto& s : dws) dw_tiles += ((s.L->out_dim + 127) / 128) * ((s.L->in_dim + 127) / 128);
    for (auto& s : dws) {
      tcg::Problem p = TP0();
      p.a = op_mn(s.gy->mn_hi, s.gy->mn_lo, (int)s.gy->kb, 0, s.gy_col0);
      p.b = op_mn(s.x->mn_hi, s.x->mn_lo, (int)s.x->kb, 0, 0);
      p.M = s.L->out_dim; p.N = s.L->in_dim; p.K = Bp;
      p.c = grad + s.L->w_off; p.ldc = s.L->in_dim; p.flags = tcg::kAccumulate;
      p.k_splits = pick_splits(p.M, p.N, p.K, dw_tiles);
      tb.add(p);
    }
  }
  PPB_CHECK_ARG((int64_t)tb.probs.size() <= t.max_probs / 2, "tensor-core problem list overflow");
  tcg::Problem* tprobs = t.probs + t.max_probs / 2;
  rc = upload_cached(net, 3, tb.probs.data(), tb.probs.size() * sizeof(tcg::Problem), tprobs, st);
  if (rc) return rc;
  rc = upload_cached(net, 4, tb.ints.data(), tb.ints.size() * sizeof(int), t.ints, st);
  if (rc) return rc;

  Builder bl;
  std::vector<int> ph_fin, ph_obs;
  int ph_obs0_dw = -1;
  if (obs_tc) {
    ph_obs0_dw = (int)bl.phases.size();
    bl.begin();
    for (int j = 0; j < D.num_obs; ++j) {
      const ppb_linear_desc& L = D.obs_ff[j].layers[0];
      bl.add(linear_dw(w.d_obs_act[j][0], L.out_dim, b->obs + obs_in_off[j], D.obs_in_total, grad + L.w_off, L.in_dim, d.B,
                       L.out_dim, L.in_dim));
    }
  }
  for (int l = D.obs_final.num_layers - 1; l >= 0 && !fused_obs && !obs_tc; --l) {
    const ppb_linear_desc& L = D.obs_final.layers[l];
    const float* X = l == 0 ? w.obs_cat : w.fin_act[l - 1];
    float* dY = (l == D.obs_final.num_layers - 1) ? w.d_obs_emb : w.d_fin_act[l];
    float* dX = l == 0 ? w.d_obs_cat : w.d_fin_act[l - 1];
    ph_fin.push_back((int)bl.phases.size());
    bl.begin();
    bl.add(linear_dw(dY, L.out_dim, X, L.in_dim, grad + L.w_off, L.in_dim, d.B, L.out_dim, L.in_dim));
    Problem px = linear_dx(dY, L.out_dim, arena + L.w_off, L.in_dim, dX, L.in_dim, d.B, L.out_dim, L.in_dim, gemm::kMaskAux);
    px.aux = X; px.ld_aux = L.in_dim;
    bl.add(px);
  }
  int max_depth = 0;
  for (int j = 0; j < D.num_obs; ++j) max_depth = D.obs_ff[j].num_layers > max_depth ? D.obs_ff[j].num_layers : max_depth;
  std::vector<int> in_off(D.num_obs), out_off(D.num_obs);
  { int ci = 0, co = 0; for (int j = 0; j < D.num_obs; ++j) { in_off[j] = ci; out_off[j] = co; ci += D.obs_ff[j].in_dim; co += D.obs_ff[j].out_dim; } }
  for (int l = max_depth - 1; l >= 0 && !fused_obs && !obs_tc; --l) {
    ph_obs.push_back((int)bl.phases.size());
    bl.begin();
    for (int j = 0; j < D.num_obs; ++j) {
      const ppb_ff_desc& ff = D.obs_ff[j];
      if (l >= ff.num_layers) continue;
      const ppb_linear_desc& L = ff.layers[l];
      bool last = (l == ff.num_layers - 1);
      const float* X = l == 0 ? b->obs + in_off[j] : w.obs_act[j][l - 1];
      int64_t ldx = l == 0 ? D.obs_in_total : ff.layers[l - 1].out_dim;
      const float* dY = last ? w.d_obs_cat + out_off[j] : w.d_obs_act[j][l];
      int64_t lddy = last ? E : L.out_dim;
      bl.add(linear_dw(dY, lddy, X, ldx, grad + L.w_off, L.in_dim, d.B, L.out_dim, L.in_dim));
      if (l > 0) {
        Problem px = linear_dx(dY, lddy, arena + L.w_off, L.in_dim, w.d_obs_act[j][l - 1], ff.layers[l - 1].out_dim, d.B, L.out_dim, L.in_dim, gemm::kMaskAux);
        px.aux = w.obs_act[j][l - 1]; px.ld_aux = ff.layers[l - 1].out_dim;
        bl.add(px);
      }
    }
  }
  Problem* dprobs = w.problems + w.max_problems / 2;
  rc = upload_and_get(net, bl, dprobs, w.max_problems / 2, st, 1);
  if (rc) return rc;

  cudaStream_t s1, s2;
  rc = side_stream(net, 0, st, &s1); if (rc) return rc;
  rc = side_stream(net, 1, st, &s2); if (rc) return rc;
  {
    bool any_splitk = false;
    for (int tt = 1; tt < d.T; ++tt) any_splitk = any_splitk || !rec_cluster[tt];
    if (any_splitk && d.T > 1)
      PPB_CUDA(cudaMemsetAsync(w.dh_rec, 0, (size_t)b->row_off_host[d.T - 1] * H * sizeof(float), st));
  }
  PPB_CUDA(cudaMemsetAsync(w.d_obs_emb, 0, (size_t)d.B * E * sizeof(float), st));
  rc = run_tc_phase_auto(tb.phases[ph_dhid], tprobs, precision, st, 2, tb); if (rc) return rc;
  rc = run_tc_phase_auto(tb.phases[ph_hw], tprobs, precision, st, 0, tb); if (rc) return rc;
  static const bool fuse_pack_on = [] { const char* e = getenv("PPB_FUSE_PACK"); return !(e && e[0] == '0'); }();
  const bool dpobs_fused = fuse_pack_on && (d.B & 127) == 0 && t.dgates.k_hi != nullptr;
  bool dpobs_packed = false;
  for (int tt = d.T - 1; tt >= 0; --tt) {
    int r0 = b->row_off_host[tt], n = b->row_off_host[tt + 1] - r0;
    int done = 0;
    if (tt + 1 < d.T) {
      if (rec_cluster[tt + 1] && net->fused_cell_bwd && bcs[tt + 1] > 1) {
        const LstmPhase& bp = bphase[tt + 1];
        const tcc::BStep* dsteps = (const tcc::BStep*)net->d_bsteps;
        const bool x3 = precision == PPB_PREC_TF32X3;
        cudaEvent_t e0 = nullptr, e1 = nullptr;
        if (g_prof.on) {
          PPB_CUDA(cudaEventCreate(&e0));
          PPB_CUDA(cudaEventCreate(&e1));
          PPB_CUDA(cudaEventRecord(e0, st));
        }
        const int cs = bcs[tt + 1];
        if (cs == 2) rc = x3 ? launch_lstm_bwd_cluster<true, 2>(bp, dsteps, st) : launch_lstm_bwd_cluster<false, 2>(bp, dsteps, st);
        else if (cs == 4) rc = x3 ? launch_lstm_bwd_cluster<true, 4>(bp, dsteps, st) : launch_lstm_bwd_cluster<false, 4>(bp, dsteps, st);
        else rc = x3 ? launch_lstm_bwd_cluster<true, 8>(bp, dsteps, st) : launch_lstm_bwd_cluster<false, 8>(bp, dsteps, st);
        if (rc) return rc;
        PPB_LAUNCH_CHECK();
        if (g_prof.on) {
          PPB_CUDA(cudaEventRecord(e1, st));
          g_prof.spans.push_back({e0, e1});
          g_prof.launches += 1;
          const gemm::Phase& ph = tb.phases[ph_rec[tt + 1]];
          for (int i = 0; i < ph.count; ++i) {
            const tcg::Problem& p = tb.probs[ph.first + i];
            g_prof.flops += 2.0 * p.M * p.N * p.K;
          }
        }
        done = b->row_off_host[tt + 2] - b->row_off_host[tt + 1];
      } else if (rec_cluster[tt + 1]) {
        rc = run_tc_phase_auto(tb.phases[ph_rec[tt + 1]], tprobs, precision, st, 0, tb, true); if (rc) return rc;
      } else {
        rc = run_tc_phase(tb.phases[ph_rec[tt + 1]], tprobs, precision, st, 1, &tb); if (rc) return rc;
      }
    }
    if (n > done) {
      if (tt == 0 && done == 0 && dpobs_fused) {
        PPB_CUDA(ppb_launch(k_cell_bwd<true>, dim3(ew_grid((int64_t)n * H)), dim3(256), 0, st, 1, 0, w.gates, w.c, w.dh, w.dh_rec,
                            w.dc, dgates, w.d_pobs, b->row_prev, b->row_next, b->row_trace, t.dgates, r0, n, H, tt, t.dpobs));
        dpobs_packed = true;
      } else {
        PPB_CUDA(ppb_launch(k_cell_bwd<false>, dim3(ew_grid((int64_t)(n - done) * H)), dim3(256), 0, st, 1, 0, w.gates, w.c, w.dh,
                            w.dh_rec, w.dc, dgates, w.d_pobs, b->row_prev, b->row_next, b->row_trace, t.dgates, r0 + done,
                            n - done, H, tt, HImg()));
      }
      PPB_LAUNCH_CHECK();
    }
  }
  rc = stream_after(net, st, s1); if (rc) return rc;
  rc = run_tc_phase(tb.phases[ph_headw], tprobs, precision, s1, 1); if (rc) return rc;
  k_head_bias_grad<<<dim3((net->dh_pad + 31) / 32 + (net->out_pad + 31) / 32, d.G), 256, 0, s1>>>(
      w.d_out, net->out_pad, w.d_hid, net->dh_pad, b->head_rows, b->group_start, b->group_addr, net->d_addrs, grad);
  PPB_LAUNCH_CHECK();
  rc = stream_after(net, st, s2); if (rc) return rc;
  const bool one_pass = S <= 4 && H4 <= 2048;
  int max_rows = 0;
  for (int s = 0; s < d.NS; ++s) max_rows = b->step_nrows_host[s] > max_rows ? b->step_nrows_host[s] : max_rows;
  if (one_pass) {
    PPB_CUDA(cudaMemsetAsync(w.d_pstep, 0, (size_t)d.NS * H4 * sizeof(float), s2));
    int slab = (d.R + 2 * PPB_NUM_SMS - 1) / (2 * PPB_NUM_SMS);
    slab = slab < 4 ? 4 : (slab > kRedSlab ? kRedSlab : slab);
    const dim3 g((max_rows + slab - 1) / slab, d.NS);
    const float* wt = d.T > 1 ? w.w_smp_t : w.p_step;
    if (H4 <= 1024)
      k_dgates_reduce<4><<<g, 256, 0, s2>>>(dgates, wt, w.smp_emb, b->values, b->step_prev_addr, b->step_row0, b->step_nrows,
                                            b->row_prev, net->d_addrs, H4, S, I, E, w.d_pstep, grad, D.w_ih_off, slab);
    else
      k_dgates_reduce<8><<<g, 256, 0, s2>>>(dgates, wt, w.smp_emb, b->values, b->step_prev_addr, b->step_row0, b->step_nrows,
                                            b->row_prev, net->d_addrs, H4, S, I, E, w.d_pstep, grad, D.w_ih_off, slab);
    PPB_LAUNCH_CHECK();
  } else {
    dim3 g((H4 + 31) / 32, d.NS);
    k_step_colsum<<<g, 256, 0, s2>>>(dgates, b->step_row0, b->step_nrows, H4, w.d_pstep);
    PPB_LAUNCH_CHECK();
  }
  PPB_CUDA(cudaMemsetAsync(w.d_embcat, 0, (size_t)d.NS * C2 * sizeof(float), s2));
  k_pstep_dx<<<dim3((C2 + 31) / 32, d.NS, 16), 256, 0, s2>>>(w.d_pstep, arena + D.w_ih_off, H4, I, E + S, C2, w.d_embcat);
  PPB_LAUNCH_CHECK();
  k_pstep_dw<<<ew_grid((int64_t)H4 * C2), 256, 0, s2>>>(w.d_pstep, w.emb_cat, d.NS, H4, I, E + S, C2, grad + D.w_ih_off);
  PPB_LAUNCH_CHECK();
  k_bias_grad<<<(H4 + 255) / 256, 256, 0, s2>>>(w.d_pstep, d.NS, H4, grad + D.b_ih_off, grad + D.b_hh_off);
  PPB_LAUNCH_CHECK();
  k_embed_scatter<<<ew_grid((int64_t)d.NS * C2), 256, 0, s2>>>(w.d_embcat, net->d_addrs, net->d_type_off, b->step_addr,
                                                               b->step_prev_addr, d.NS, D.type_dim, D.addr_dim, grad);
  PPB_LAUNCH_CHECK();
  if (d.T > 1 && !one_pass) {
    const int slab = 64;
    k_smp_bwd_seg<<<dim3((max_rows + slab - 1) / slab, d.NS), 128, 0, s2>>>(dgates, w.w_smp_t, w.smp_emb, b->values,
                                                                           b->step_prev_addr, b->step_row0, b->step_nrows,
                                                                           b->row_prev, net->d_addrs, H4, S, slab, grad);
    PPB_LAUNCH_CHECK();
    int rpb = 1024;
    dim3 g((H4 + 255) / 256, (d.R + rpb - 1) / rpb);
    k_wsmp_grad<<<g, 256, 0, s2>>>(dgates, w.smp_emb, d.R, H4, S, I, E, grad + D.w_ih_off, rpb);
    PPB_LAUNCH_CHECK();
  }
  if (!dpobs_packed) {
    PPB_CUDA(ppb_launch(k_pack_rows, dim3(dim3((d.B + 127) / 128, 64)), dim3(256), 0, st, 1, 0, w.d_pobs, d.B, H4, H4, t.dpobs));
    PPB_LAUNCH_CHECK();
  }
  rc = run_tc_phase(tb.phases[ph_lstm_w], tprobs, precision, st, 1, &tb); if (rc) return rc;
  if (fused_obs) {
    rc = obs_fused_bwd(D, arena, grad, b->obs, d.B, w, st); if (rc) return rc;
    rc = stream_after(net, s1, st); if (rc) return rc;
    return stream_after(net, s2, st);
  }
  if (obs_tc) {
    PPB_CUDA(ppb_launch(k_pack_rows_masked, dim3(dim3((d.B + 127) / 128, 4)), dim3(256), 0, st, 1, 0, w.d_obs_emb, w.obs_emb, d.B, E, E, t.g_emb));
    PPB_LAUNCH_CHECK();
    for (int ph : ph_bobs_dx) { rc = run_tc_phase_auto(tb.phases[ph], tprobs, precision, st, 2, tb); if (rc) return rc; }
    rc = run_tc_phase(tb.phases[ph_bobs_dw], tprobs, precision, st, 1); if (rc) return rc;
    for (int l = 0; l < D.obs_final.num_layers; ++l) {
      const ppb_linear_desc& L = D.obs_final.layers[l];
      const float* dY = (l == D.obs_final.num_layers - 1) ? w.d_obs_emb : w.d_fin_act[l];
      k_colsum_gather<<<dim3((L.out_dim + 31) / 32, 8), 256, 0, st>>>(dY, L.out_dim, nullptr, d.B, L.out_dim, grad + L.b_off);
      PPB_LAUNCH_CHECK();
    }
    for (int j = 0; j < D.num_obs; ++j) {
      const ppb_ff_desc& ff = D.obs_ff[j];
      for (int l = 0; l < ff.num_layers; ++l) {
        const ppb_linear_desc& L = ff.layers[l];
        const bool last = l == ff.num_layers - 1;
        const float* dY = last ? w.d_obs_cat + obs_out_off[j] : w.d_obs_act[j][l];
        k_colsum_gather<<<dim3((L.out_dim + 31) / 32, 8), 256, 0, st>>>(dY, last ? E : L.out_dim, nullptr, d.B, L.out_dim,
                                                                        grad + L.b_off);
        PPB_LAUNCH_CHECK();
      }
    }
    rc = run_phase(bl.phases[ph_obs0_dw], dprobs, st); if (rc) return rc;
    rc = stream_after(net, s1, st); if (rc) return rc;
    return stream_after(net, s2, st);
  }
  k_mask_nonpos<<<ew_grid((int64_t)d.B * E), 256, 0, st>>>(w.d_obs_emb, w.obs_emb, (int64_t)d.B * E);
  PPB_LAUNCH_CHECK();
  for (size_t k = 0; k < ph_fin.size(); ++k) {
    int l = D.obs_final.num_layers - 1 - (int)k;
    const ppb_linear_desc& L = D.obs_final.layers[l];
    float* dY = (l == D.obs_final.num_layers - 1) ? w.d_obs_emb : w.d_fin_act[l];
    k_colsum_gather<<<dim3((L.out_dim + 31) / 32, 8), 256, 0, st>>>(dY, L.out_dim, nullptr, d.B, L.out_dim, grad + L.b_off);
    PPB_LAUNCH_CHECK();
    rc = run_phase(bl.phases[ph_fin[k]], dprobs, st); if (rc) return rc;
  }
  for (size_t k = 0; k < ph_obs.size(); ++k) {
    int l = max_depth - 1 - (int)k;
    for (int j = 0; j < D.num_obs; ++j) {
      const ppb_ff_desc& ff = D.obs_ff[j];
      if (l >= ff.num_layers) continue;
      const ppb_linear_desc& L = ff.layers[l];
      bool last = (l == ff.num_layers - 1);
      const float* dY = last ? w.d_obs_cat + out_off[j] : w.d_obs_act[j][l];
      int64_t lddy = last ? E : L.out_dim;
      k_colsum_gather<<<dim3((L.out_dim + 31) / 32, 8), 256, 0, st>>>(dY, lddy, nullptr, d.B, L.out_dim, grad + L.b_off);
      PPB_LAUNCH_CHECK();
    }
    rc = run_phase(bl.phases[ph_obs[k]], dprobs, st); if (rc) return rc;
  }
  rc = stream_after(net, s1, st); if (rc) return rc;
  return stream_after(net, s2, st);
}

}
```

### pyprob_b200/csrc/obs_mlp.cuh

```cuda
#pragma once
#include "common.cuh"
#include "tc.cuh"

namespace obsmlp {

constexpr int TB = 4;
constexpr int WMAX = 256;
constexpr int LD = WMAX + 1;
constexpr int NC = 64;
constexpr int kThreads = 256;

struct Bufs {
  float* obs_act[PPB_MAX_OBS][PPB_MAX_FF_LAYERS];
  float* obs_cat;
  float* fin_act[PPB_MAX_FF_LAYERS];
  float* obs_emb;
  float* emb_k_hi = nullptr; float* emb_k_lo = nullptr; float* emb_mn_hi = nullptr; float* emb_mn_lo = nullptr;
  long long emb_kb = 0;
};

struct Net {
  int num_obs, obs_in_total, E;
  ppb_ff_desc obs_ff[PPB_MAX_OBS];
  ppb_ff_desc obs_final;
};

inline size_t smem_bytes() { return (size_t)(3 * TB * LD + WMAX * (NC + 1)) * sizeof(float); }

__device__ __forceinline__ void dense_fwd(const float (*in_s)[LD], int in_dim, const float* __restrict__ W,
                                          const float* __restrict__ b, int out_dim, float (*out_s)[LD], int out_col0,
                                          float* ws, float* gout, int64_t ldg, int gcol0, int r0, int B) {
  const int tid = threadIdx.x;
  for (int n0 = 0; n0 < out_dim; n0 += NC) {
    const int nc = out_dim - n0 < NC ? out_dim - n0 : NC;
    for (int idx = tid; idx < nc * in_dim; idx += kThreads) {
      int nn = idx / in_dim, k = idx - nn * in_dim;
      ws[k * (NC + 1) + nn] = __ldg(W + (int64_t)(n0 + nn) * in_dim + k);
    }
    __syncthreads();
    for (int o = tid; o < TB * NC; o += kThreads) {
      int r = o / NC, nn = o % NC;
      if (nn < nc) {
        float acc = __ldg(b + n0 + nn);
#pragma unroll 4
        for (int k = 0; k < in_dim; ++k) acc = fmaf(in_s[r][k], ws[k * (NC + 1) + nn], acc);
        acc = fmaxf(acc, 0.0f);
        out_s[r][out_col0 + n0 + nn] = acc;
        if (r0 + r < B) gout[(int64_t)(r0 + r) * ldg + gcol0 + n0 + nn] = acc;
      }
    }
    __syncthreads();
  }
}

__global__ void __launch_bounds__(kThreads) k_fwd(Net net, const float* __restrict__ arena, const float* __restrict__ obs,
                                                   int B, Bufs bufs) {
  extern __shared__ float smem[];
  float (*cat)[LD] = reinterpret_cast<float (*)[LD]>(smem);
  float (*pa)[LD] = reinterpret_cast<float (*)[LD]>(smem + TB * LD);
  float (*pb)[LD] = reinterpret_cast<float (*)[LD]>(smem + 2 * TB * LD);
  float* ws = smem + 3 * TB * LD;
  const int r0 = blockIdx.x * TB, tid = threadIdx.x;
  int in_off = 0, out_off = 0;
  for (int j = 0; j < net.num_obs; ++j) {
    const ppb_ff_desc& ff = net.obs_ff[j];
    for (int idx = tid; idx < TB * ff.in_dim; idx += kThreads) {
      int r = idx / ff.in_dim, k = idx % ff.in_dim;
      pa[r][k] = (r0 + r < B) ? __ldg(obs + (int64_t)(r0 + r) * net.obs_in_total + in_off + k) : 0.0f;
    }
    __syncthreads();
    float (*cur)[LD] = pa;
    float (*nxt)[LD] = pb;
    for (int l = 0; l < ff.num_layers; ++l) {
      const ppb_linear_desc& L = ff.layers[l];
      const bool last = l == ff.num_layers - 1;
      if (last) dense_fwd(cur, L.in_dim, arena + L.w_off, arena + L.b_off, L.out_dim, cat, out_off, ws, bufs.obs_cat, net.E, out_off, r0, B);
      else dense_fwd(cur, L.in_dim, arena + L.w_off, arena + L.b_off, L.out_dim, nxt, 0, ws, bufs.obs_act[j][l], L.out_dim, 0, r0, B);
      float (*t)[LD] = cur; cur = nxt; nxt = t;
    }
    in_off += ff.in_dim;
    out_off += ff.out_dim;
  }
  float (*cur)[LD] = cat;
  float (*nxt)[LD] = pa;
  for (int l = 0; l < net.obs_final.num_layers; ++l) {
    const ppb_linear_desc& L = net.obs_final.layers[l];
    const bool last = l == net.obs_final.num_layers - 1;
    dense_fwd(cur, L.in_dim, arena + L.w_off, arena + L.b_off, L.out_dim, nxt, 0, ws, last ? bufs.obs_emb : bufs.fin_act[l],
              L.out_dim, 0, r0, B);
    cur = nxt;
    nxt = (nxt == pa) ? pb : pa;
  }
}

__device__ __forceinline__ void dense_bwd(const float (*dy_s)[LD], int dy_col0, int out_dim, const float* __restrict__ x,
                                          int64_t ldx, int xcol0, int in_dim, const float* __restrict__ W,
                                          float* __restrict__ dW, float* __restrict__ db, float (*x_s)[LD],
                                          float (*dx_s)[LD], bool want_dx, int r0, int B) {
  const int tid = threadIdx.x;
  for (int idx = tid; idx < TB * in_dim; idx += kThreads) {
    int r = idx / in_dim, k = idx % in_dim;
    x_s[r][k] = (r0 + r < B) ? __ldg(x + (int64_t)(r0 + r) * ldx + xcol0 + k) : 0.0f;
  }
  __syncthreads();
  for (int idx = tid; idx < out_dim * in_dim; idx += kThreads) {
    int n = idx / in_dim, k = idx - n * in_dim;
    float s = 0.0f;
#pragma unroll
    for (int r = 0; r < TB; ++r) s = fmaf(dy_s[r][dy_col0 + n], x_s[r][k], s);
    if (s != 0.0f) atomicAdd(dW + idx, s);
  }
  for (int n = tid; n < out_dim; n += kThreads) {
    float s = 0.0f;
#pragma unroll
    for (int r = 0; r < TB; ++r) s += dy_s[r][dy_col0 + n];
    if (s != 0.0f) atomicAdd(db + n, s);
  }
  if (want_dx) {
    for (int idx = tid; idx < TB * in_dim; idx += kThreads) {
      int r = idx / in_dim, k = idx - r * in_dim;
      float s = 0.0f;
      for (int n = 0; n < out_dim; ++n) s = fmaf(dy_s[r][dy_col0 + n], __ldg(W + (int64_t)n * in_dim + k), s);
      dx_s[r][k] = x_s[r][k] > 0.0f ? s : 0.0f;
    }
  }
  __syncthreads();
}

__global__ void __launch_bounds__(kThreads) k_bwd(Net net, const float* __restrict__ arena, float* __restrict__ grad,
                                                   const float* __restrict__ obs, const float* __restrict__ d_obs_emb,
                                                   int B, Bufs bufs) {
  extern __shared__ float smem[];
  float (*da)[LD] = reinterpret_cast<float (*)[LD]>(smem);
  float (*dbuf)[LD] = reinterpret_cast<float (*)[LD]>(smem + TB * LD);
  float (*xs)[LD] = reinterpret_cast<float (*)[LD]>(smem + 2 * TB * LD);
  const int r0 = blockIdx.x * TB, tid = threadIdx.x, E = net.E;
  for (int idx = tid; idx < TB * E; idx += kThreads) {
    int r = idx / E, k = idx % E;
    float g = 0.0f;
    if (r0 + r < B) {
      int64_t o = (int64_t)(r0 + r) * E + k;
      g = bufs.obs_emb[o] > 0.0f ? d_obs_emb[o] : 0.0f;
    }
    da[r][k] = g;
  }
  __syncthreads();
  float (*cur)[LD] = da;
  float (*nxt)[LD] = dbuf;
  for (int l = net.obs_final.num_layers - 1; l >= 0; --l) {
    const ppb_linear_desc& L = net.obs_final.layers[l];
    const float* x = l == 0 ? bufs.obs_cat : bufs.fin_act[l - 1];
    dense_bwd(cur, 0, L.out_dim, x, L.in_dim, 0, L.in_dim, arena + L.w_off, grad + L.w_off, grad + L.b_off, xs, nxt, true, r0, B);
    float (*t)[LD] = cur; cur = nxt; nxt = t;
  }
  float (*dcat)[LD] = cur;
  float (*tmp)[LD] = nxt;
  float (*tmp2)[LD] = reinterpret_cast<float (*)[LD]>(smem + 3 * TB * LD);
  int in_off = 0, out_off = 0;
  for (int j = 0; j < net.num_obs; ++j) {
    const ppb_ff_desc& ff = net.obs_ff[j];
    const float (*dy)[LD] = dcat;
    int dy_col0 = out_off;
    float (*o1)[LD] = tmp;
    float (*o2)[LD] = tmp2;
    for (int l = ff.num_layers - 1; l >= 0; --l) {
      const ppb_linear_desc& L = ff.layers[l];
      const float* x = l == 0 ? obs : bufs.obs_act[j][l - 1];
      int64_t ldx = l == 0 ? net.obs_in_total : ff.layers[l - 1].out_dim;
      int xcol0 = l == 0 ? in_off : 0;
      dense_bwd(dy, dy_col0, L.out_dim, x, ldx, xcol0, L.in_dim, arena + L.w_off, grad + L.w_off, grad + L.b_off, xs, o1,
                l > 0, r0, B);
      dy = o1; dy_col0 = 0;
      float (*t)[LD] = o1; o1 = o2; o2 = t;
    }
    in_off += ff.in_dim;
    out_off += ff.out_dim;
  }
}

inline size_t smem_bytes_bwd() { return (size_t)(4 * TB * LD) * sizeof(float); }

constexpr int W2 = 96;
constexpr int TPW = 1;
constexpr int kWarps = 8;

struct DBufs {
  float* d_obs_act[PPB_MAX_OBS][PPB_MAX_FF_LAYERS];
  float* d_obs_cat;
  float* d_fin_act[PPB_MAX_FF_LAYERS];
  float* d_obs_emb;
};

__host__ __device__ inline int layer_floats(const ppb_linear_desc& L) { return L.out_dim * (L.in_dim | 1) + L.out_dim; }
__host__ __device__ inline int weights_floats(const Net& net) {
  int n = 0;
  for (int j = 0; j < net.num_obs; ++j)
    for (int l = 0; l < net.obs_ff[j].num_layers; ++l) n += layer_floats(net.obs_ff[j].layers[l]);
  for (int l = 0; l < net.obs_final.num_layers; ++l) n += layer_floats(net.obs_final.layers[l]);
  return n;
}
inline size_t smem_bytes2(const Net& net) { return (size_t)(weights_floats(net) + kWarps * 3 * W2) * sizeof(float); }

__device__ __forceinline__ void cp_async4(float* smem_dst, const float* gmem_src) {
  asm volatile("cp.async.ca.shared.global [%0], [%1], 4;" ::"r"((uint32_t)__cvta_generic_to_shared(smem_dst)), "l"(gmem_src)
               : "memory");
}
__device__ __forceinline__ void cp_async_wait_all() {
  asm volatile("cp.async.commit_group;" ::: "memory");
  asm volatile("cp.async.wait_group 0;" ::: "memory");
}
__device__ __forceinline__ float* stage_layer(float* dst, const float* __restrict__ arena, const ppb_linear_desc& L) {
  const int pitch = L.in_dim | 1, nw = L.out_dim * L.in_dim;
  for (int idx = threadIdx.x; idx < nw; idx += blockDim.x) {
    int n = idx / L.in_dim, k = idx - n * L.in_dim;
    cp_async4(dst + n * pitch + k, arena + L.w_off + idx);
  }
  float* bias = dst + L.out_dim * pitch;
  for (int n = threadIdx.x; n < L.out_dim; n += blockDim.x) cp_async4(bias + n, arena + L.b_off + n);
  return bias + L.out_dim;
}

__device__ __forceinline__ void warp_dense_fwd(const float* in, int in_dim, const float* w, int out_dim, float* out,
                                               int out_col0, float* gout, int lane) {
  const int pitch = in_dim | 1;
  const float* bias = w + out_dim * pitch;
  const bool p0 = lane < out_dim, p1 = lane + 32 < out_dim, p2 = lane + 64 < out_dim;
  const float* r0 = w + (p0 ? lane : 0) * pitch;
  const float* r1 = w + (p1 ? lane + 32 : 0) * pitch;
  const float* r2 = w + (p2 ? lane + 64 : 0) * pitch;
  float a0 = p0 ? bias[lane] : 0.f, a1 = p1 ? bias[lane + 32] : 0.f, a2 = p2 ? bias[lane + 64] : 0.f;
  if (out_dim <= 32) {
#pragma unroll 4
    for (int k = 0; k < in_dim; ++k) a0 = fmaf(in[k], r0[k], a0);
  } else if (out_dim <= 64) {
#pragma unroll 4
    for (int k = 0; k < in_dim; ++k) { const float x = in[k]; a0 = fmaf(x, r0[k], a0); a1 = fmaf(x, r1[k], a1); }
  } else {
#pragma unroll 4
    for (int k = 0; k < in_dim; ++k) { const float x = in[k]; a0 = fmaf(x, r0[k], a0); a1 = fmaf(x, r1[k], a1); a2 = fmaf(x, r2[k], a2); }
  }
  a0 = fmaxf(a0, 0.f); a1 = fmaxf(a1, 0.f); a2 = fmaxf(a2, 0.f);
  if (p0) { out[out_col0 + lane] = a0; gout[lane] = a0; }
  if (p1) { out[out_col0 + lane + 32] = a1; gout[lane + 32] = a1; }
  if (p2) { out[out_col0 + lane + 64] = a2; gout[lane + 64] = a2; }
  __syncwarp();
}

__global__ void __launch_bounds__(kWarps * 32) k_fwd2(Net net, const float* __restrict__ arena,
                                                      const float* __restrict__ obs, int B, int traces_per_cta, Bufs bufs) {
  ppb_pdl_trigger();
  extern __shared__ float smem[];
  float* p = smem;
  const float* w_obs[PPB_MAX_OBS][PPB_MAX_FF_LAYERS];
  const float* w_fin[PPB_MAX_FF_LAYERS];
  for (int j = 0; j < net.num_obs; ++j)
    for (int l = 0; l < net.obs_ff[j].num_layers; ++l) { w_obs[j][l] = p; p = stage_layer(p, arena, net.obs_ff[j].layers[l]); }
  for (int l = 0; l < net.obs_final.num_layers; ++l) { w_fin[l] = p; p = stage_layer(p, arena, net.obs_final.layers[l]); }
  const int warp = threadIdx.x >> 5, lane = threadIdx.x & 31;
  float* cat = p + warp * 3 * W2;
  float* va = cat + W2;
  float* vb = va + W2;
  cp_async_wait_all();
  __syncthreads();
  const int t0 = blockIdx.x * traces_per_cta;
  for (int tr = t0 + warp; tr < t0 + traces_per_cta && tr < B; tr += kWarps) {
    int in_off = 0, out_off = 0;
    for (int j = 0; j < net.num_obs; ++j) {
      const ppb_ff_desc& ff = net.obs_ff[j];
      float* cur = va;
      float* nxt = vb;
      for (int k = lane; k < ff.in_dim; k += 32) cur[k] = __ldg(obs + (int64_t)tr * net.obs_in_total + in_off + k);
      __syncwarp();
      for (int l = 0; l < ff.num_layers; ++l) {
        const ppb_linear_desc& L = ff.layers[l];
        const bool last = l == ff.num_layers - 1;
        if (last) warp_dense_fwd(cur, L.in_dim, w_obs[j][l], L.out_dim, cat, out_off, bufs.obs_cat + (int64_t)tr * net.E + out_off, lane);
        else warp_dense_fwd(cur, L.in_dim, w_obs[j][l], L.out_dim, nxt, 0, bufs.obs_act[j][l] + (int64_t)tr * L.out_dim, lane);
        float* t = cur; cur = nxt; nxt = t;
      }
      in_off += ff.in_dim;
      out_off += ff.out_dim;
    }
    float* cur = cat;
    float* nxt = va;
    for (int l = 0; l < net.obs_final.num_layers; ++l) {
      const ppb_linear_desc& L = net.obs_final.layers[l];
      const bool last = l == net.obs_final.num_layers - 1;
      warp_dense_fwd(cur, L.in_dim, w_fin[l], L.out_dim, nxt, 0,
                     (last ? bufs.obs_emb : bufs.fin_act[l]) + (int64_t)tr * L.out_dim, lane);
      float* t = cur; cur = nxt; nxt = (t == cat) ? vb : t;
    }
    if (bufs.emb_k_hi) {
      for (int k = lane; k < net.E; k += 32) {
        float hi, lo;
        tc::split_tf32(cur[k], hi, lo);
        const int64_t ok = tc::packed_offset(tr, k, bufs.emb_kb);
        bufs.emb_k_hi[ok] = hi;
        if (bufs.emb_k_lo) bufs.emb_k_lo[ok] = lo;
        if (bufs.emb_mn_hi) {
          const int64_t om = tc::packed_offset_mn(tr, k, bufs.emb_kb);
          bufs.emb_mn_hi[om] = hi;
          if (bufs.emb_mn_lo) bufs.emb_mn_lo[om] = lo;
        }
      }
    }
    __syncwarp();
  }
}

__device__ __forceinline__ void warp_dense_dx(const float* dy, int out_dim, const float* w, int in_dim,
                                              const float* __restrict__ x, float* dx, float* gdx, int lane) {
  const int pitch = in_dim | 1;
  const bool p0 = lane < in_dim, p1 = lane + 32 < in_dim, p2 = lane + 64 < in_dim;
  const float x0 = p0 ? __ldg(x + lane) : 0.f, x1 = p1 ? __ldg(x + lane + 32) : 0.f, x2 = p2 ? __ldg(x + lane + 64) : 0.f;
  const float* c0 = w + (p0 ? lane : 0);
  const float* c1 = w + (p1 ? lane + 32 : 0);
  const float* c2 = w + (p2 ? lane + 64 : 0);
  float a0 = 0.f, a1 = 0.f, a2 = 0.f;
  if (in_dim <= 32) {
#pragma unroll 4
    for (int n = 0; n < out_dim; ++n) a0 = fmaf(dy[n], c0[n * pitch], a0);
  } else if (in_dim <= 64) {
#pragma unroll 4
    for (int n = 0; n < out_dim; ++n) { const float g = dy[n]; a0 = fmaf(g, c0[n * pitch], a0); a1 = fmaf(g, c1[n * pitch], a1); }
  } else {
#pragma unroll 4
    for (int n = 0; n < out_dim; ++n) { const float g = dy[n]; a0 = fmaf(g, c0[n * pitch], a0); a1 = fmaf(g, c1[n * pitch], a1); a2 = fmaf(g, c2[n * pitch], a2); }
  }
  if (p0) { a0 = x0 > 0.f ? a0 : 0.f; dx[lane] = a0; gdx[lane] = a0; }
  if (p1) { a1 = x1 > 0.f ? a1 : 0.f; dx[lane + 32] = a1; gdx[lane + 32] = a1; }
  if (p2) { a2 = x2 > 0.f ? a2 : 0.f; dx[lane + 64] = a2; gdx[lane + 64] = a2; }
  __syncwarp();
}

__global__ void __launch_bounds__(kWarps * 32) k_bwd2_dx(Net net, const float* __restrict__ arena, int B, int traces_per_cta,
                                                         Bufs bufs, DBufs dbufs) {
  ppb_pdl_trigger();
  ppb_pdl_wait();
  extern __shared__ float smem[];
  float* p = smem;
  const float* w_obs[PPB_MAX_OBS][PPB_MAX_FF_LAYERS];
  const float* w_fin[PPB_MAX_FF_LAYERS];
  for (int j = 0; j < net.num_obs; ++j)
    for (int l = 0; l < net.obs_ff[j].num_layers; ++l) {
      w_obs[j][l] = p;
      if (l > 0) p = stage_layer(p, arena, net.obs_ff[j].layers[l]);
    }
  for (int l = 0; l < net.obs_final.num_layers; ++l) { w_fin[l] = p; p = stage_layer(p, arena, net.obs_final.layers[l]); }
  const int warp = threadIdx.x >> 5, lane = threadIdx.x & 31, E = net.E;
  float* va = p + warp * 3 * W2;
  float* vb = va + W2;
  float* vc = vb + W2;
  cp_async_wait_all();
  __syncthreads();
  const int t0 = blockIdx.x * traces_per_cta;
  for (int tr = t0 + warp; tr < t0 + traces_per_cta && tr < B; tr += kWarps) {
    for (int k = lane; k < E; k += 32) {
      int64_t o = (int64_t)tr * E + k;
      float g = bufs.obs_emb[o] > 0.f ? dbufs.d_obs_emb[o] : 0.f;
      va[k] = g;
      dbufs.d_obs_emb[o] = g;
    }
    __syncwarp();
    float* cur = va;
    float* nxt = vb;
    for (int l = net.obs_final.num_layers - 1; l >= 0; --l) {
      const ppb_linear_desc& L = net.obs_final.layers[l];
      const float* x = (l == 0 ? bufs.obs_cat : bufs.fin_act[l - 1]) + (int64_t)tr * L.in_dim;
      float* gdx = (l == 0 ? dbufs.d_obs_cat : dbufs.d_fin_act[l - 1]) + (int64_t)tr * L.in_dim;
      warp_dense_dx(cur, L.out_dim, w_fin[l], L.in_dim, x, nxt, gdx, lane);
      float* t = cur; cur = nxt; nxt = t;
    }
    float* dcat = cur;
    float* scratch = nxt;
    int out_off = 0;
    for (int j = 0; j < net.num_obs; ++j) {
      const ppb_ff_desc& ff = net.obs_ff[j];
      const float* dy = dcat + out_off;
      float* o1 = scratch;
      float* o2 = vc;
      for (int l = ff.num_layers - 1; l >= 1; --l) {
        const ppb_linear_desc& L = ff.layers[l];
        const float* x = bufs.obs_act[j][l - 1] + (int64_t)tr * L.in_dim;
        warp_dense_dx(dy, L.out_dim, w_obs[j][l], L.in_dim, x, o1, dbufs.d_obs_act[j][l - 1] + (int64_t)tr * L.in_dim, lane);
        dy = o1;
        float* t = o1; o1 = o2; o2 = t;
      }
      out_off += ff.out_dim;
    }
    __syncwarp();
  }
}

struct DwLayer { const float* dy; const float* x; int ldy, ldx, out_dim, in_dim, start, pad_; int64_t w_off, b_off; };
struct DwTable { int n_layers, total; DwLayer layer[PPB_MAX_OBS * PPB_MAX_FF_LAYERS + PPB_MAX_FF_LAYERS]; };

__global__ void __launch_bounds__(256) k_dw(DwTable tab, int B, int b_chunk, float* __restrict__ grad) {
  ppb_pdl_trigger();
  ppb_pdl_wait();
  __shared__ float part[8][33];
  const int lane = threadIdx.x & 31, warp = threadIdx.x >> 5;
  const int idx = blockIdx.x * 32 + lane;
  float s = 0.f;
  int li = 0, e = 0, nw = 0;
  const bool live = idx < tab.total;
  if (live) {
    while (li + 1 < tab.n_layers && tab.layer[li + 1].start <= idx) ++li;
    const DwLayer& L = tab.layer[li];
    e = idx - L.start;
    nw = L.out_dim * L.in_dim;
    const int b0 = blockIdx.y * b_chunk, b1 = min(B, b0 + b_chunk);
    if (e < nw) {
      const int n = e / L.in_dim, k = e - n * L.in_dim;
      const float* dy = L.dy + n;
      const float* x = L.x + k;
#pragma unroll 8
      for (int b = b0 + warp; b < b1; b += 8) s = fmaf(__ldg(dy + (int64_t)b * L.ldy), __ldg(x + (int64_t)b * L.ldx), s);
    } else {
      const float* dy = L.dy + (e - nw);
#pragma unroll 8
      for (int b = b0 + warp; b < b1; b += 8) s += __ldg(dy + (int64_t)b * L.ldy);
    }
  }
  part[warp][lane] = s;
  __syncthreads();
  if (warp == 0 && live) {
    float t = 0.f;
#pragma unroll
    for (int w = 0; w < 8; ++w) t += part[w][lane];
    const DwLayer& L = tab.layer[li];
    if (t != 0.f) atomicAdd(grad + (e < nw ? L.w_off + e : L.b_off + (e - nw)), t);
  }
}

}
```

Baseline: 1.459 million.

## Rewrite obs MLP as plan-driven fused kernels and fuse pstep backward

Replaces the observation MLP forward and backward kernels with plan-driven versions that process tiles of traces in shared memory. The backward now computes weight gradients per CTA and reduces them across a thread-block cluster through distributed shared memory before issuing atomics, replacing the separate dx and dw kernels. It also merges the pstep dx, dw, bias and embedding-scatter kernels into one launch and adds a z-split to the head bias gradient. Workspace buffers are reordered so a single memset clears d_pstep through d_obs_emb. The aim is fewer launches and less global traffic, at the cost of larger shared-memory use and more complex indexing.

```diff
diff --git a/pyprob_b200/csrc/net.cu b/pyprob_b200/csrc/net.cu
--- a/pyprob_b200/csrc/net.cu
+++ b/pyprob_b200/csrc/net.cu
@@ -145,9 +145,9 @@
   w.dh_rec = take((int64_t)d.R * H);
   w.dc = take((int64_t)d.R * H);
   w.d_pobs = take((int64_t)d.B * 4 * H);
-  w.d_pstep = take((int64_t)d.NS * 4 * H);
   w.d_smp = take((int64_t)d.R * S);
   w.d_embcat = take((int64_t)d.NS * C2);
+  w.d_pstep = take((int64_t)d.NS * 4 * H);
   w.d_obs_emb = take((int64_t)d.B * E);
   for (int l = 0; l + 1 < D.obs_final.num_layers; ++l) w.d_fin_act[l] = take((int64_t)d.B * D.obs_final.layers[l].out_dim);
   w.d_obs_cat = take((int64_t)d.B * E);
diff --git a/pyprob_b200/csrc/net_tc.inc b/pyprob_b200/csrc/net_tc.inc
--- a/pyprob_b200/csrc/net_tc.inc
+++ b/pyprob_b200/csrc/net_tc.inc
@@ -442,12 +442,64 @@
 
 inline int pad128(int n) { return (n + 127) / 128 * 128; }
 
-inline obsmlp::Net obs_net_of(const ppb_net_desc& D) {
-  obsmlp::Net n;
-  n.num_obs = D.num_obs; n.obs_in_total = D.obs_in_total; n.E = D.obs_dim;
-  for (int j = 0; j < PPB_MAX_OBS; ++j) n.obs_ff[j] = D.obs_ff[j];
-  n.obs_final = D.obs_final;
-  return n;
+inline obsmlp::Plan obs_plan_of(const ppb_net_desc& D, const Ws* w, const float* obs) {
+  obsmlp::Plan P;
+  memset(&P, 0, sizeof(P));
+  const int E = D.obs_dim;
+  P.E = E;
+  int nf = 0;
+  auto add_layer = [&](const ppb_linear_desc& L) -> obsmlp::Layer& {
+    obsmlp::Layer& o = P.L[P.n_layers++];
+    o.in_dim = L.in_dim; o.out_dim = L.out_dim; o.w_off = L.w_off; o.b_off = L.b_off;
+    o.pitch = (L.in_dim & 3) ? L.in_dim : ((L.in_dim & 7) ? L.in_dim : L.in_dim + 4);
+    o.sw = nf;
+    nf += (L.out_dim * o.pitch + L.out_dim + 3) & ~3;
+    o.part = P.part_floats;
+    P.part_floats += L.out_dim * L.in_dim + L.out_dim;
+    return o;
+  };
+  std::vector<int> first(D.num_obs);
+  int in_off = 0;
+  for (int j = 0; j < D.num_obs; ++j) {
+    const ppb_ff_desc& ff = D.obs_ff[j];
+    first[j] = P.n_layers;
+    for (int l = 0; l < ff.num_layers; ++l) {
+      obsmlp::Layer& o = add_layer(ff.layers[l]);
+      o.xoff = P.A; P.A += o.in_dim;
+      if (l + 1 < ff.num_layers) { o.dzoff = P.Dz; P.Dz += o.out_dim; }
+      o.dxoff = l == 0 ? -1 : P.L[P.n_layers - 2].dzoff;
+      o.x = l == 0 ? obs + in_off : (w ? w->obs_act[j][l - 1] : nullptr);
+      o.ldx = l == 0 ? D.obs_in_total : ff.layers[l - 1].out_dim;
+      if (l + 1 < ff.num_layers) { o.y = w ? w->obs_act[j][l] : nullptr; o.ldy = o.out_dim; }
+    }
+    in_off += ff.in_dim;
+  }
+  const int cat = P.A, dcat = P.Dz;
+  P.A += E; P.Dz += E;
+  int out_off = 0;
+  for (int j = 0; j < D.num_obs; ++j) {
+    obsmlp::Layer& o = P.L[first[j] + D.obs_ff[j].num_layers - 1];
+    o.yoff = cat + out_off; o.dzoff = dcat + out_off;
+    o.y = w ? w->obs_cat + out_off : nullptr; o.ldy = E;
+    out_off += D.obs_ff[j].out_dim;
+  }
+  for (int j = 0; j < D.num_obs; ++j)
+    for (int l = 0; l + 1 < D.obs_ff[j].num_layers; ++l) P.L[first[j] + l].yoff = P.L[first[j] + l + 1].xoff;
+  const int nfin = D.obs_final.num_layers;
+  for (int l = 0; l < nfin; ++l) {
+    const bool last = l == nfin - 1;
+    obsmlp::Layer& o = add_layer(D.obs_final.layers[l]);
+    if (l == 0) o.xoff = cat;
+    o.yoff = P.A; P.A += o.out_dim;
+    o.dzoff = P.Dz; P.Dz += o.out_dim;
+    o.dxoff = l == 0 ? dcat : P.L[P.n_layers - 2].dzoff;
+    o.x = l == 0 ? (w ? w->obs_cat : nullptr) : (w ? w->fin_act[l - 1] : nullptr);
+    o.ldx = o.in_dim;
+    o.y = w ? (last ? w->obs_emb : w->fin_act[l]) : nullptr; o.ldy = o.out_dim;
+    if (l > 0) o.xoff = P.L[P.n_layers - 2].yoff;
+  }
+  P.w_floats = nf;
+  return P;
 }
 inline bool obs_fused_ok(const ppb_net_desc& D, int B) {
   constexpr int kFuseMaxWidth = obsmlp::W2;
@@ -458,89 +510,44 @@
   for (int l = 0; l < D.obs_final.num_layers; ++l)
     if (D.obs_final.layers[l].in_dim > kFuseMaxWidth || D.obs_final.layers[l].out_dim > kFuseMaxWidth) return false;
   (void)B;
-  return obsmlp::smem_bytes2(obs_net_of(D)) <= 200 * 1024;
-}
-inline obsmlp::Bufs obs_bufs_of(const Ws& w) {
-  obsmlp::Bufs b;
-  for (int j = 0; j < PPB_MAX_OBS; ++j)
-    for (int l = 0; l < PPB_MAX_FF_LAYERS; ++l) b.obs_act[j][l] = w.obs_act[j][l];
-  b.obs_cat = w.obs_cat;
-  for (int l = 0; l < PPB_MAX_FF_LAYERS; ++l) b.fin_act[l] = w.fin_act[l];
-  b.obs_emb = w.obs_emb;
-  return b;
-}
-inline obsmlp::DBufs obs_dbufs_of(const Ws& w) {
-  obsmlp::DBufs b;
-  for (int j = 0; j < PPB_MAX_OBS; ++j)
-    for (int l = 0; l < PPB_MAX_FF_LAYERS; ++l) b.d_obs_act[j][l] = w.d_obs_act[j][l];
-  b.d_obs_cat = w.d_obs_cat;
-  for (int l = 0; l < PPB_MAX_FF_LAYERS; ++l) b.d_fin_act[l] = w.d_fin_act[l];
-  b.d_obs_emb = w.d_obs_emb;
-  return b;
-}
-inline int obs_traces_per_cta(int B) {
-  int t = (B + PPB_NUM_SMS - 1) / PPB_NUM_SMS;
-  t = (t + obsmlp::kWarps - 1) / obsmlp::kWarps * obsmlp::kWarps;
-  return t < obsmlp::kWarps ? obsmlp::kWarps : t;
+  const obsmlp::Plan P = obs_plan_of(D, nullptr, nullptr);
+  return obsmlp::smem_fwd(P) <= obsmlp::kMaxSmem && obsmlp::smem_bwd(P) <= obsmlp::kMaxSmem;
+}
+int obs_set_smem_limits() {
+  static bool attr = false;
+  if (!attr) {
+    PPB_CUDA(cudaFuncSetAttribute(obsmlp::k_fwd, cudaFuncAttributeMaxDynamicSharedMemorySize, (int)obsmlp::kMaxSmem));
+    PPB_CUDA(cudaFuncSetAttribute(obsmlp::k_bwd, cudaFuncAttributeMaxDynamicSharedMemorySize, (int)obsmlp::kMaxSmem));
+    attr = true;
+  }
+  return PPB_OK;
 }
 int obs_fused_fwd(const ppb_net_desc& D, const float* arena, const float* obs, int B, const Ws& w, cudaStream_t st,
                   const HImg* emb_img = nullptr) {
-  static bool attr = false;
-  if (!attr) {
-    PPB_CUDA(cudaFuncSetAttribute(obsmlp::k_fwd2, cudaFuncAttributeMaxDynamicSharedMemorySize, 200 * 1024));
-    PPB_CUDA(cudaFuncSetAttribute(obsmlp::k_bwd2_dx, cudaFuncAttributeMaxDynamicSharedMemorySize, 200 * 1024));
-    attr = true;
-  }
-  const obsmlp::Net n = obs_net_of(D);
-  const int tpc = obs_traces_per_cta(B);
-  obsmlp::Bufs bufs = obs_bufs_of(w);
+  int rc = obs_set_smem_limits();
+  if (rc) return rc;
+  obsmlp::Plan P = obs_plan_of(D, &w, obs);
   if (emb_img) {
-    bufs.emb_k_hi = emb_img->k_hi; bufs.emb_k_lo = emb_img->k_lo; bufs.emb_mn_hi = emb_img->mn_hi; bufs.emb_mn_lo = emb_img->mn_lo;
-    bufs.emb_kb = emb_img->kb;
-  }
-  obsmlp::k_fwd2<<<(B + tpc - 1) / tpc, obsmlp::kWarps * 32, obsmlp::smem_bytes2(n), st>>>(n, arena, obs, B, tpc, bufs);
+    P.emb_k_hi = emb_img->k_hi; P.emb_k_lo = emb_img->k_lo; P.emb_mn_hi = emb_img->mn_hi; P.emb_mn_lo = emb_img->mn_lo;
+    P.emb_kb = emb_img->kb;
+  }
+  const int tpc = (B + PPB_NUM_SMS - 1) / PPB_NUM_SMS;
+  obsmlp::k_fwd<<<(B + tpc - 1) / tpc, obsmlp::kThreads, obsmlp::smem_fwd(P), st>>>(P, arena, B, tpc);
   PPB_LAUNCH_CHECK();
   return PPB_OK;
 }
 int obs_fused_bwd(const ppb_net_desc& D, const float* arena, float* grad, const float* obs, int B, const Ws& w,
                   cudaStream_t st) {
-  const obsmlp::Net n = obs_net_of(D);
-  const int tpc = obs_traces_per_cta(B);
-  PPB_CUDA(ppb_launch(obsmlp::k_bwd2_dx, dim3((B + tpc - 1) / tpc), dim3(obsmlp::kWarps * 32), obsmlp::smem_bytes2(n), st, 2,
-                      0, n, arena, B, tpc, obs_bufs_of(w), obs_dbufs_of(w)));
-  PPB_LAUNCH_CHECK();
-  obsmlp::DwTable tab;
-  memset(&tab, 0, sizeof(tab));
-  int total = 0;
-  auto add = [&](const float* dy, int ldy, const float* x, int ldx, const ppb_linear_desc& L) {
-    obsmlp::DwLayer& e = tab.layer[tab.n_layers++];
-    e.dy = dy; e.ldy = ldy; e.x = x; e.ldx = ldx; e.out_dim = L.out_dim; e.in_dim = L.in_dim;
-    e.w_off = L.w_off; e.b_off = L.b_off; e.start = total;
-    total += L.out_dim * L.in_dim + L.out_dim;
-  };
-  const int E = D.obs_dim;
-  for (int l = 0; l < D.obs_final.num_layers; ++l) {
-    const ppb_linear_desc& L = D.obs_final.layers[l];
-    const bool last = l == D.obs_final.num_layers - 1;
-    add(last ? w.d_obs_emb : w.d_fin_act[l], L.out_dim, l == 0 ? w.obs_cat : w.fin_act[l - 1], L.in_dim, L);
-  }
-  int in_off = 0, out_off = 0;
-  for (int j = 0; j < D.num_obs; ++j) {
-    const ppb_ff_desc& ff = D.obs_ff[j];
-    for (int l = 0; l < ff.num_layers; ++l) {
-      const ppb_linear_desc& L = ff.layers[l];
-      const bool last = l == ff.num_layers - 1;
-      const float* dy = last ? w.d_obs_cat + out_off : w.d_obs_act[j][l];
-      const float* x = l == 0 ? obs + in_off : w.obs_act[j][l - 1];
-      add(dy, last ? E : L.out_dim, x, l == 0 ? D.obs_in_total : ff.layers[l - 1].out_dim, L);
-    }
-    in_off += ff.in_dim;
-    out_off += ff.out_dim;
-  }
-  tab.total = total;
-  const int b_chunk = 512;
-  PPB_CUDA(ppb_launch(obsmlp::k_dw, dim3((total + 31) / 32, (B + b_chunk - 1) / b_chunk), dim3(256), 0, st, 2, 0, tab, B,
-                      b_chunk, grad));
+  int rc = obs_set_smem_limits();
+  if (rc) return rc;
+  const obsmlp::Plan P = obs_plan_of(D, &w, obs);
+  constexpr int kMaxCtas = 16 * obsmlp::kCluster;
+  int tpc = (B + kMaxCtas - 1) / kMaxCtas;
+  tpc = tpc < obsmlp::kMT ? obsmlp::kMT : tpc;
+  int ctas = (B + tpc - 1) / tpc;
+  ctas = (ctas + obsmlp::kCluster - 1) / obsmlp::kCluster * obsmlp::kCluster;
+  PPB_CUDA(ppb_launch(obsmlp::k_bwd, dim3(ctas), dim3(obsmlp::kThreads), obsmlp::smem_bwd(P), st, 2, obsmlp::kCluster, P, arena,
+                      (const float*)w.d_obs_emb, grad, B, tpc));
   PPB_LAUNCH_CHECK();
   return PPB_OK;
 }
@@ -571,7 +578,7 @@
   const int s0 = group_start[g], cnt = group_start[g + 1] - s0;
   float s = 0.0f;
   if (n < width)
-    for (int m = slice; m < cnt; m += 8) s += src[(int64_t)head_rows[s0 + m] * ld + n];
+    for (int m = blockIdx.z * 8 + slice; m < cnt; m += 8 * gridDim.z) s += src[(int64_t)head_rows[s0 + m] * ld + n];
   part[slice][lane] = s;
   __syncthreads();
   if (slice == 0 && n < width) {
@@ -595,32 +602,54 @@
     if (lane == 0) p_step[o] = s + b_ih[col] + b_hh[col];
   }
 }
-__global__ void __launch_bounds__(256) k_pstep_dx(const float* __restrict__ d_pstep, const float* __restrict__ w_ih,
-                                                   int H4, int I, int off, int C2, float* __restrict__ d_embcat) {
-  __shared__ float part[8][33];
-  const int st = blockIdx.y, lane = threadIdx.x & 31, slice = threadIdx.x >> 5;
-  const int j = blockIdx.x * 32 + lane;
-  float s = 0.0f;
-  if (j < C2)
-    for (int col = blockIdx.z * 8 + slice; col < H4; col += 8 * gridDim.z)
-      s = fmaf(d_pstep[(int64_t)st * H4 + col], w_ih[(int64_t)col * I + off + j], s);
-  part[slice][lane] = s;
-  __syncthreads();
-  if (slice == 0 && j < C2) {
-    float t = 0.0f;
+__global__ void __launch_bounds__(256) k_pstep_bwd(const float* __restrict__ d_pstep, const float* __restrict__ w_ih,
+                                                    const float* __restrict__ emb_cat, const ppb_addr_desc* __restrict__ addrs,
+                                                    const int64_t* __restrict__ type_off, const int* __restrict__ step_addr,
+                                                    const int* __restrict__ step_prev, int NS, int H4, int I, int off, int td,
+                                                    int ad, int zsplit, int nx, float* __restrict__ grad, int64_t w_ih_off,
+                                                    int64_t b_ih_off, int64_t b_hh_off) {
+  const int C2 = 2 * (td + ad);
+  if ((int)blockIdx.x < nx) {
+    __shared__ float part[8][33];
+    const int jbs = (C2 + 31) / 32;
+    const int jb = blockIdx.x % jbs, st = (blockIdx.x / jbs) % NS, z = blockIdx.x / (jbs * NS);
+    const int lane = threadIdx.x & 31, slice = threadIdx.x >> 5;
+    const int j = jb * 32 + lane;
+    float s = 0.0f;
+    if (j < C2)
+      for (int col = z * 8 + slice; col < H4; col += 8 * zsplit)
+        s = fmaf(d_pstep[(int64_t)st * H4 + col], __ldg(w_ih + (int64_t)col * I + off + j), s);
+    part[slice][lane] = s;
+    __syncthreads();
+    if (slice == 0 && j < C2) {
+      float t = 0.0f;
 #pragma unroll
-    for (int k = 0; k < 8; ++k) t += part[k][lane];
-    atomicAdd(d_embcat + (int64_t)st * C2 + j, t);
-  }
-}
-__global__ void __launch_bounds__(256) k_pstep_dw(const float* __restrict__ d_pstep, const float* __restrict__ emb_cat,
-                                                   int NS, int H4, int I, int off, int C2, float* __restrict__ dw_ih) {
-  for (int64_t e = (int64_t)blockIdx.x * blockDim.x + threadIdx.x; e < (int64_t)H4 * C2;
-       e += (int64_t)gridDim.x * blockDim.x) {
-    int col = (int)(e / C2), j = (int)(e % C2);
-    float s = 0.0f;
-    for (int st = 0; st < NS; ++st) s = fmaf(d_pstep[(int64_t)st * H4 + col], emb_cat[(int64_t)st * C2 + j], s);
-    dw_ih[(int64_t)col * I + off + j] += s;
+      for (int k = 0; k < 8; ++k) t += part[k][lane];
+      const int which = j < td + ad ? step_prev[st] : step_addr[st];
+      const int jj = j < td + ad ? j : j - (td + ad);
+      if (which >= 0 && t != 0.0f) {
+        const ppb_addr_desc& a = addrs[which];
+        if (jj < td) atomicAdd(grad + type_off[a.type_id] + jj, t);
+        else atomicAdd(grad + a.addr_emb_off + (jj - td), t);
+      }
+    }
+    return;
+  }
+  const int64_t nwe = (int64_t)H4 * C2;
+  for (int64_t e = (int64_t)(blockIdx.x - nx) * blockDim.x + threadIdx.x; e < nwe + H4;
+       e += (int64_t)(gridDim.x - nx) * blockDim.x) {
+    if (e < nwe) {
+      const int col = (int)(e / C2), j = (int)(e % C2);
+      float s = 0.0f;
+      for (int st = 0; st < NS; ++st) s = fmaf(d_pstep[(int64_t)st * H4 + col], emb_cat[(int64_t)st * C2 + j], s);
+      grad[w_ih_off + (int64_t)col * I + off + j] += s;
+    } else {
+      const int col = (int)(e - nwe);
+      float s = 0.0f;
+      for (int st = 0; st < NS; ++st) s += d_pstep[(int64_t)st * H4 + col];
+      grad[b_ih_off + col] += s;
+      grad[b_hh_off + col] += s;
+    }
   }
 }
 
@@ -1365,7 +1394,7 @@
     if (any_splitk && d.T > 1)
       PPB_CUDA(cudaMemsetAsync(w.dh_rec, 0, (size_t)b->row_off_host[d.T - 1] * H * sizeof(float), st));
   }
-  PPB_CUDA(cudaMemsetAsync(w.d_obs_emb, 0, (size_t)d.B * E * sizeof(float), st));
+  PPB_CUDA(cudaMemsetAsync(w.d_pstep, 0, (size_t)((const char*)(w.d_obs_emb + (int64_t)d.B * E) - (const char*)w.d_pstep), st));
   rc = run_tc_phase_auto(tb.phases[ph_dhid], tprobs, precision, st, 2, tb); if (rc) return rc;
   rc = run_tc_phase_auto(tb.phases[ph_hw], tprobs, precision, st, 0, tb); if (rc) return rc;
   static const bool fuse_pack_on = [] { const char* e = getenv("PPB_FUSE_PACK"); return !(e && e[0] == '0'); }();
@@ -1423,15 +1452,23 @@
   }
   rc = stream_after(net, st, s1); if (rc) return rc;
   rc = run_tc_phase(tb.phases[ph_headw], tprobs, precision, s1, 1); if (rc) return rc;
-  k_head_bias_grad<<<dim3((net->dh_pad + 31) / 32 + (net->out_pad + 31) / 32, d.G), 256, 0, s1>>>(
-      w.d_out, net->out_pad, w.d_hid, net->dh_pad, b->head_rows, b->group_start, b->group_addr, net->d_addrs, grad);
-  PPB_LAUNCH_CHECK();
+  {
+    const int cb = (net->dh_pad + 31) / 32 + (net->out_pad + 31) / 32;
+    int max_rows = 0;
+    for (int g = 0; g < d.G; ++g) max_rows = b->group_start_host[g + 1] - b->group_start_host[g] > max_rows ? b->group_start_host[g + 1] - b->group_start_host[g] : max_rows;
+    int zs = PPB_NUM_SMS / (cb * d.G);
+    const int zmax = (max_rows + 63) / 64;
+    zs = zs > zmax ? zmax : zs;
+    zs = zs < 1 ? 1 : zs;
+    k_head_bias_grad<<<dim3(cb, d.G, zs), 256, 0, s1>>>(w.d_out, net->out_pad, w.d_hid, net->dh_pad, b->head_rows, b->group_start,
+                                                         b->group_addr, net->d_addrs, grad);
+    PPB_LAUNCH_CHECK();
+  }
   rc = stream_after(net, st, s2); if (rc) return rc;
   const bool one_pass = S <= 4 && H4 <= 2048;
   int max_rows = 0;
   for (int s = 0; s < d.NS; ++s) max_rows = b->step_nrows_host[s] > max_rows ? b->step_nrows_host[s] : max_rows;
   if (one_pass) {
-    PPB_CUDA(cudaMemsetAsync(w.d_pstep, 0, (size_t)d.NS * H4 * sizeof(float), s2));
     int slab = (d.R + 2 * PPB_NUM_SMS - 1) / (2 * PPB_NUM_SMS);
     slab = slab < 4 ? 4 : (slab > kRedSlab ? kRedSlab : slab);
     const dim3 g((max_rows + slab - 1) / slab, d.NS);
@@ -1448,16 +1485,17 @@
     k_step_colsum<<<g, 256, 0, s2>>>(dgates, b->step_row0, b->step_nrows, H4, w.d_pstep);
     PPB_LAUNCH_CHECK();
   }
-  PPB_CUDA(cudaMemsetAsync(w.d_embcat, 0, (size_t)d.NS * C2 * sizeof(float), s2));
-  k_pstep_dx<<<dim3((C2 + 31) / 32, d.NS, 16), 256, 0, s2>>>(w.d_pstep, arena + D.w_ih_off, H4, I, E + S, C2, w.d_embcat);
-  PPB_LAUNCH_CHECK();
-  k_pstep_dw<<<ew_grid((int64_t)H4 * C2), 256, 0, s2>>>(w.d_pstep, w.emb_cat, d.NS, H4, I, E + S, C2, grad + D.w_ih_off);
-  PPB_LAUNCH_CHECK();
-  k_bias_grad<<<(H4 + 255) / 256, 256, 0, s2>>>(w.d_pstep, d.NS, H4, grad + D.b_ih_off, grad + D.b_hh_off);
-  PPB_LAUNCH_CHECK();
-  k_embed_scatter<<<ew_grid((int64_t)d.NS * C2), 256, 0, s2>>>(w.d_embcat, net->d_addrs, net->d_type_off, b->step_addr,
-                                                               b->step_prev_addr, d.NS, D.type_dim, D.addr_dim, grad);
-  PPB_LAUNCH_CHECK();
+  {
+    const int jbs = (C2 + 31) / 32;
+    int zsplit = PPB_NUM_SMS / 2 / (jbs * d.NS);
+    zsplit = zsplit < 1 ? 1 : (zsplit > 16 ? 16 : zsplit);
+    const int nx = jbs * d.NS * zsplit;
+    const int nw = (int)(((int64_t)H4 * C2 + H4 + 255) / 256);
+    k_pstep_bwd<<<nx + nw, 256, 0, s2>>>(w.d_pstep, arena + D.w_ih_off, w.emb_cat, net->d_addrs, net->d_type_off, b->step_addr,
+                                         b->step_prev_addr, d.NS, H4, I, E + S, D.type_dim, D.addr_dim, zsplit, nx, grad,
+                                         D.w_ih_off, D.b_ih_off, D.b_hh_off);
+    PPB_LAUNCH_CHECK();
+  }
   if (d.T > 1 && !one_pass) {
     const int slab = 64;
     k_smp_bwd_seg<<<dim3((max_rows + slab - 1) / slab, d.NS), 128, 0, s2>>>(dgates, w.w_smp_t, w.smp_emb, b->values,
diff --git a/pyprob_b200/csrc/obs_mlp.cuh b/pyprob_b200/csrc/obs_mlp.cuh
--- a/pyprob_b200/csrc/obs_mlp.cuh
+++ b/pyprob_b200/csrc/obs_mlp.cuh
@@ -1,206 +1,47 @@
 #pragma once
 #include "common.cuh"
 #include "tc.cuh"
+#include "tc_cluster.cuh"
 
 namespace obsmlp {
 
-constexpr int TB = 4;
-constexpr int WMAX = 256;
-constexpr int LD = WMAX + 1;
-constexpr int NC = 64;
+constexpr int W2 = 96;
 constexpr int kThreads = 256;
-
-struct Bufs {
-  float* obs_act[PPB_MAX_OBS][PPB_MAX_FF_LAYERS];
-  float* obs_cat;
-  float* fin_act[PPB_MAX_FF_LAYERS];
-  float* obs_emb;
-  float* emb_k_hi = nullptr; float* emb_k_lo = nullptr; float* emb_mn_hi = nullptr; float* emb_mn_lo = nullptr;
-  long long emb_kb = 0;
+constexpr int kSlices = 8;
+constexpr int kRows = kThreads / kSlices;
+constexpr int kMT = 4;
+constexpr int kCluster = 8;
+constexpr int kMaxLayers = PPB_MAX_OBS * PPB_MAX_FF_LAYERS + PPB_MAX_FF_LAYERS;
+constexpr size_t kMaxSmem = 227 * 1024;
+
+struct Layer {
+  int in_dim, out_dim;
+  int sw, pitch;
+  int xoff, yoff;
+  int dzoff, dxoff;
+  int part;
+  int64_t w_off, b_off;
+  float* y; int ldy;
+  const float* x; int ldx;
 };
 
-struct Net {
-  int num_obs, obs_in_total, E;
-  ppb_ff_desc obs_ff[PPB_MAX_OBS];
-  ppb_ff_desc obs_final;
+struct Plan {
+  int n_layers;
+  int A, Dz;
+  int w_floats, part_floats;
+  int E;
+  Layer L[kMaxLayers];
+  float* emb_k_hi; float* emb_k_lo; float* emb_mn_hi; float* emb_mn_lo;
+  long long emb_kb;
 };
 
-inline size_t smem_bytes() { return (size_t)(3 * TB * LD + WMAX * (NC + 1)) * sizeof(float); }
-
-__device__ __forceinline__ void dense_fwd(const float (*in_s)[LD], int in_dim, const float* __restrict__ W,
-                                          const float* __restrict__ b, int out_dim, float (*out_s)[LD], int out_col0,
-                                          float* ws, float* gout, int64_t ldg, int gcol0, int r0, int B) {
-  const int tid = threadIdx.x;
-  for (int n0 = 0; n0 < out_dim; n0 += NC) {
-    const int nc = out_dim - n0 < NC ? out_dim - n0 : NC;
-    for (int idx = tid; idx < nc * in_dim; idx += kThreads) {
-      int nn = idx / in_dim, k = idx - nn * in_dim;
-      ws[k * (NC + 1) + nn] = __ldg(W + (int64_t)(n0 + nn) * in_dim + k);
-    }
-    __syncthreads();
-    for (int o = tid; o < TB * NC; o += kThreads) {
-      int r = o / NC, nn = o % NC;
-      if (nn < nc) {
-        float acc = __ldg(b + n0 + nn);
-#pragma unroll 4
-        for (int k = 0; k < in_dim; ++k) acc = fmaf(in_s[r][k], ws[k * (NC + 1) + nn], acc);
-        acc = fmaxf(acc, 0.0f);
-        out_s[r][out_col0 + n0 + nn] = acc;
-        if (r0 + r < B) gout[(int64_t)(r0 + r) * ldg + gcol0 + n0 + nn] = acc;
-      }
-    }
-    __syncthreads();
-  }
-}
-
-__global__ void __launch_bounds__(kThreads) k_fwd(Net net, const float* __restrict__ arena, const float* __restrict__ obs,
-                                                   int B, Bufs bufs) {
-  extern __shared__ float smem[];
-  float (*cat)[LD] = reinterpret_cast<float (*)[LD]>(smem);
-  float (*pa)[LD] = reinterpret_cast<float (*)[LD]>(smem + TB * LD);
-  float (*pb)[LD] = reinterpret_cast<float (*)[LD]>(smem + 2 * TB * LD);
-  float* ws = smem + 3 * TB * LD;
-  const int r0 = blockIdx.x * TB, tid = threadIdx.x;
-  int in_off = 0, out_off = 0;
-  for (int j = 0; j < net.num_obs; ++j) {
-    const ppb_ff_desc& ff = net.obs_ff[j];
-    for (int idx = tid; idx < TB * ff.in_dim; idx += kThreads) {
-      int r = idx / ff.in_dim, k = idx % ff.in_dim;
-      pa[r][k] = (r0 + r < B) ? __ldg(obs + (int64_t)(r0 + r) * net.obs_in_total + in_off + k) : 0.0f;
-    }
-    __syncthreads();
-    float (*cur)[LD] = pa;
-    float (*nxt)[LD] = pb;
-    for (int l = 0; l < ff.num_layers; ++l) {
-      const ppb_linear_desc& L = ff.layers[l];
-      const bool last = l == ff.num_layers - 1;
-      if (last) dense_fwd(cur, L.in_dim, arena + L.w_off, arena + L.b_off, L.out_dim, cat, out_off, ws, bufs.obs_cat, net.E, out_off, r0, B);
-      else dense_fwd(cur, L.in_dim, arena + L.w_off, arena + L.b_off, L.out_dim, nxt, 0, ws, bufs.obs_act[j][l], L.out_dim, 0, r0, B);
-      float (*t)[LD] = cur; cur = nxt; nxt = t;
-    }
-    in_off += ff.in_dim;
-    out_off += ff.out_dim;
-  }
-  float (*cur)[LD] = cat;
-  float (*nxt)[LD] = pa;
-  for (int l = 0; l < net.obs_final.num_layers; ++l) {
-    const ppb_linear_desc& L = net.obs_final.layers[l];
-    const bool last = l == net.obs_final.num_layers - 1;
-    dense_fwd(cur, L.in_dim, arena + L.w_off, arena + L.b_off, L.out_dim, nxt, 0, ws, last ? bufs.obs_emb : bufs.fin_act[l],
-              L.out_dim, 0, r0, B);
-    cur = nxt;
-    nxt = (nxt == pa) ? pb : pa;
-  }
-}
-
-__device__ __forceinline__ void dense_bwd(const float (*dy_s)[LD], int dy_col0, int out_dim, const float* __restrict__ x,
-                                          int64_t ldx, int xcol0, int in_dim, const float* __restrict__ W,
-                                          float* __restrict__ dW, float* __restrict__ db, float (*x_s)[LD],
-                                          float (*dx_s)[LD], bool want_dx, int r0, int B) {
-  const int tid = threadIdx.x;
-  for (int idx = tid; idx < TB * in_dim; idx += kThreads) {
-    int r = idx / in_dim, k = idx % in_dim;
-    x_s[r][k] = (r0 + r < B) ? __ldg(x + (int64_t)(r0 + r) * ldx + xcol0 + k) : 0.0f;
-  }
-  __syncthreads();
-  for (int idx = tid; idx < out_dim * in_dim; idx += kThreads) {
-    int n = idx / in_dim, k = idx - n * in_dim;
-    float s = 0.0f;
-#pragma unroll
-    for (int r = 0; r < TB; ++r) s = fmaf(dy_s[r][dy_col0 + n], x_s[r][k], s);
-    if (s != 0.0f) atomicAdd(dW + idx, s);
-  }
-  for (int n = tid; n < out_dim; n += kThreads) {
-    float s = 0.0f;
-#pragma unroll
-    for (int r = 0; r < TB; ++r) s += dy_s[r][dy_col0 + n];
-    if (s != 0.0f) atomicAdd(db + n, s);
-  }
-  if (want_dx) {
-    for (int idx = tid; idx < TB * in_dim; idx += kThreads) {
-      int r = idx / in_dim, k = idx - r * in_dim;
-      float s = 0.0f;
-      for (int n = 0; n < out_dim; ++n) s = fmaf(dy_s[r][dy_col0 + n], __ldg(W + (int64_t)n * in_dim + k), s);
-      dx_s[r][k] = x_s[r][k] > 0.0f ? s : 0.0f;
-    }
-  }
-  __syncthreads();
-}
-
-__global__ void __launch_bounds__(kThreads) k_bwd(Net net, const float* __restrict__ arena, float* __restrict__ grad,
-                                                   const float* __restrict__ obs, const float* __restrict__ d_obs_emb,
-                                                   int B, Bufs bufs) {
-  extern __shared__ float smem[];
-  float (*da)[LD] = reinterpret_cast<float (*)[LD]>(smem);
-  float (*dbuf)[LD] = reinterpret_cast<float (*)[LD]>(smem + TB * LD);
-  float (*xs)[LD] = reinterpret_cast<float (*)[LD]>(smem + 2 * TB * LD);
-  const int r0 = blockIdx.x * TB, tid = threadIdx.x, E = net.E;
-  for (int idx = tid; idx < TB * E; idx += kThreads) {
-    int r = idx / E, k = idx % E;
-    float g = 0.0f;
-    if (r0 + r < B) {
-      int64_t o = (int64_t)(r0 + r) * E + k;
-      g = bufs.obs_emb[o] > 0.0f ? d_obs_emb[o] : 0.0f;
-    }
-    da[r][k] = g;
-  }
-  __syncthreads();
-  float (*cur)[LD] = da;
-  float (*nxt)[LD] = dbuf;
-  for (int l = net.obs_final.num_layers - 1; l >= 0; --l) {
-    const ppb_linear_desc& L = net.obs_final.layers[l];
-    const float* x = l == 0 ? bufs.obs_cat : bufs.fin_act[l - 1];
-    dense_bwd(cur, 0, L.out_dim, x, L.in_dim, 0, L.in_dim, arena + L.w_off, grad + L.w_off, grad + L.b_off, xs, nxt, true, r0, B);
-    float (*t)[LD] = cur; cur = nxt; nxt = t;
-  }
-  float (*dcat)[LD] = cur;
-  float (*tmp)[LD] = nxt;
-  float (*tmp2)[LD] = reinterpret_cast<float (*)[LD]>(smem + 3 * TB * LD);
-  int in_off = 0, out_off = 0;
-  for (int j = 0; j < net.num_obs; ++j) {
-    const ppb_ff_desc& ff = net.obs_ff[j];
-    const float (*dy)[LD] = dcat;
-    int dy_col0 = out_off;
-    float (*o1)[LD] = tmp;
-    float (*o2)[LD] = tmp2;
-    for (int l = ff.num_layers - 1; l >= 0; --l) {
-      const ppb_linear_desc& L = ff.layers[l];
-      const float* x = l == 0 ? obs : bufs.obs_act[j][l - 1];
-      int64_t ldx = l == 0 ? net.obs_in_total : ff.layers[l - 1].out_dim;
-      int xcol0 = l == 0 ? in_off : 0;
-      dense_bwd(dy, dy_col0, L.out_dim, x, ldx, xcol0, L.in_dim, arena + L.w_off, grad + L.w_off, grad + L.b_off, xs, o1,
-                l > 0, r0, B);
-      dy = o1; dy_col0 = 0;
-      float (*t)[LD] = o1; o1 = o2; o2 = t;
-    }
-    in_off += ff.in_dim;
-    out_off += ff.out_dim;
-  }
-}
-
-inline size_t smem_bytes_bwd() { return (size_t)(4 * TB * LD) * sizeof(float); }
-
-constexpr int W2 = 96;
-constexpr int TPW = 1;
-constexpr int kWarps = 8;
-
-struct DBufs {
-  float* d_obs_act[PPB_MAX_OBS][PPB_MAX_FF_LAYERS];
-  float* d_obs_cat;
-  float* d_fin_act[PPB_MAX_FF_LAYERS];
-  float* d_obs_emb;
-};
-
-__host__ __device__ inline int layer_floats(const ppb_linear_desc& L) { return L.out_dim * (L.in_dim | 1) + L.out_dim; }
-__host__ __device__ inline int weights_floats(const Net& net) {
-  int n = 0;
-  for (int j = 0; j < net.num_obs; ++j)
-    for (int l = 0; l < net.obs_ff[j].num_layers; ++l) n += layer_floats(net.obs_ff[j].layers[l]);
-  for (int l = 0; l < net.obs_final.num_layers; ++l) n += layer_floats(net.obs_final.layers[l]);
-  return n;
-}
-inline size_t smem_bytes2(const Net& net) { return (size_t)(weights_floats(net) + kWarps * 3 * W2) * sizeof(float); }
-
+inline size_t smem_fwd(const Plan& p) { return (size_t)(p.w_floats + kMT * p.A) * sizeof(float); }
+inline size_t smem_bwd(const Plan& p) { return (size_t)(p.w_floats + p.part_floats + kMT * (p.A + p.Dz)) * sizeof(float); }
+
+__device__ __forceinline__ void cp_async16(float* smem_dst, const float* gmem_src) {
+  asm volatile("cp.async.cg.shared.global [%0], [%1], 16;" ::"r"((uint32_t)__cvta_generic_to_shared(smem_dst)), "l"(gmem_src)
+               : "memory");
+}
 __device__ __forceinline__ void cp_async4(float* smem_dst, const float* gmem_src) {
   asm volatile("cp.async.ca.shared.global [%0], [%1], 4;" ::"r"((uint32_t)__cvta_generic_to_shared(smem_dst)), "l"(gmem_src)
                : "memory");
@@ -209,228 +50,225 @@
   asm volatile("cp.async.commit_group;" ::: "memory");
   asm volatile("cp.async.wait_group 0;" ::: "memory");
 }
-__device__ __forceinline__ float* stage_layer(float* dst, const float* __restrict__ arena, const ppb_linear_desc& L) {
-  const int pitch = L.in_dim | 1, nw = L.out_dim * L.in_dim;
-  for (int idx = threadIdx.x; idx < nw; idx += blockDim.x) {
-    int n = idx / L.in_dim, k = idx - n * L.in_dim;
-    cp_async4(dst + n * pitch + k, arena + L.w_off + idx);
-  }
-  float* bias = dst + L.out_dim * pitch;
-  for (int n = threadIdx.x; n < L.out_dim; n += blockDim.x) cp_async4(bias + n, arena + L.b_off + n);
-  return bias + L.out_dim;
-}
-
-__device__ __forceinline__ void warp_dense_fwd(const float* in, int in_dim, const float* w, int out_dim, float* out,
-                                               int out_col0, float* gout, int lane) {
-  const int pitch = in_dim | 1;
+
+__device__ __forceinline__ void stage_layer(float* smem, const float* __restrict__ arena, const Layer& L) {
+  const int in_dim = L.in_dim, out_dim = L.out_dim, pitch = L.pitch;
+  float* dst = smem + L.sw;
+  const float* src = arena + L.w_off;
+  const float* bsrc = arena + L.b_off;
+  if ((in_dim & 3) == 0) {
+    const int q = in_dim >> 2, nq = out_dim * q;
+    for (int c = threadIdx.x; c < nq; c += kThreads) {
+      const int n = c / q, k4 = c - n * q;
+      cp_async16(dst + n * pitch + 4 * k4, src + 4 * c);
+    }
+  } else {
+    const int nw = out_dim * in_dim;
+    for (int c = threadIdx.x; c < nw; c += kThreads) cp_async4(dst + c, src + c);
+  }
+  float* bias = dst + out_dim * pitch;
+  for (int n = threadIdx.x; n < out_dim; n += kThreads) cp_async4(bias + n, bsrc + n);
+}
+__device__ __forceinline__ void load_rows(float* dst, int pitch, const float* src, int64_t ld, int tr0, int nt, int width) {
+  for (int idx = threadIdx.x; idx < nt * width; idx += kThreads) {
+    const int t = idx / width, k = idx - t * width;
+    cp_async4(dst + t * pitch + k, src + (int64_t)(tr0 + t) * ld + k);
+  }
+}
+
+__device__ __forceinline__ float group_sum(float v) {
+  v += __shfl_xor_sync(0xffffffffu, v, 4);
+  v += __shfl_xor_sync(0xffffffffu, v, 2);
+  v += __shfl_xor_sync(0xffffffffu, v, 1);
+  return v;
+}
+__device__ __forceinline__ float pick(const float (&a)[kMT], int i) {
+  float r = a[0];
+#pragma unroll
+  for (int t = 1; t < kMT; ++t) r = i == t ? a[t] : r;
+  return r;
+}
+
+__device__ __forceinline__ void layer_fwd(const Plan& P, const Layer& L, const float* smem, float* act, int tr0, int nt,
+                                          bool last) {
+  const int g = threadIdx.x / kSlices, s = threadIdx.x % kSlices;
+  const int in_dim = L.in_dim, out_dim = L.out_dim, pitch = L.pitch, A = P.A, ldy = L.ldy;
+  const float* w = smem + L.sw;
   const float* bias = w + out_dim * pitch;
-  const bool p0 = lane < out_dim, p1 = lane + 32 < out_dim, p2 = lane + 64 < out_dim;
-  const float* r0 = w + (p0 ? lane : 0) * pitch;
-  const float* r1 = w + (p1 ? lane + 32 : 0) * pitch;
-  const float* r2 = w + (p2 ? lane + 64 : 0) * pitch;
-  float a0 = p0 ? bias[lane] : 0.f, a1 = p1 ? bias[lane + 32] : 0.f, a2 = p2 ? bias[lane + 64] : 0.f;
-  if (out_dim <= 32) {
-#pragma unroll 4
-    for (int k = 0; k < in_dim; ++k) a0 = fmaf(in[k], r0[k], a0);
-  } else if (out_dim <= 64) {
-#pragma unroll 4
-    for (int k = 0; k < in_dim; ++k) { const float x = in[k]; a0 = fmaf(x, r0[k], a0); a1 = fmaf(x, r1[k], a1); }
-  } else {
-#pragma unroll 4
-    for (int k = 0; k < in_dim; ++k) { const float x = in[k]; a0 = fmaf(x, r0[k], a0); a1 = fmaf(x, r1[k], a1); a2 = fmaf(x, r2[k], a2); }
-  }
-  a0 = fmaxf(a0, 0.f); a1 = fmaxf(a1, 0.f); a2 = fmaxf(a2, 0.f);
-  if (p0) { out[out_col0 + lane] = a0; gout[lane] = a0; }
-  if (p1) { out[out_col0 + lane + 32] = a1; gout[lane + 32] = a1; }
-  if (p2) { out[out_col0 + lane + 64] = a2; gout[lane + 64] = a2; }
-  __syncwarp();
-}
-
-__global__ void __launch_bounds__(kWarps * 32) k_fwd2(Net net, const float* __restrict__ arena,
-                                                      const float* __restrict__ obs, int B, int traces_per_cta, Bufs bufs) {
-  ppb_pdl_trigger();
-  extern __shared__ float smem[];
-  float* p = smem;
-  const float* w_obs[PPB_MAX_OBS][PPB_MAX_FF_LAYERS];
-  const float* w_fin[PPB_MAX_FF_LAYERS];
-  for (int j = 0; j < net.num_obs; ++j)
-    for (int l = 0; l < net.obs_ff[j].num_layers; ++l) { w_obs[j][l] = p; p = stage_layer(p, arena, net.obs_ff[j].layers[l]); }
-  for (int l = 0; l < net.obs_final.num_layers; ++l) { w_fin[l] = p; p = stage_layer(p, arena, net.obs_final.layers[l]); }
-  const int warp = threadIdx.x >> 5, lane = threadIdx.x & 31;
-  float* cat = p + warp * 3 * W2;
-  float* va = cat + W2;
-  float* vb = va + W2;
-  cp_async_wait_all();
-  __syncthreads();
-  const int t0 = blockIdx.x * traces_per_cta;
-  for (int tr = t0 + warp; tr < t0 + traces_per_cta && tr < B; tr += kWarps) {
-    int in_off = 0, out_off = 0;
-    for (int j = 0; j < net.num_obs; ++j) {
-      const ppb_ff_desc& ff = net.obs_ff[j];
-      float* cur = va;
-      float* nxt = vb;
-      for (int k = lane; k < ff.in_dim; k += 32) cur[k] = __ldg(obs + (int64_t)tr * net.obs_in_total + in_off + k);
-      __syncwarp();
-      for (int l = 0; l < ff.num_layers; ++l) {
-        const ppb_linear_desc& L = ff.layers[l];
-        const bool last = l == ff.num_layers - 1;
-        if (last) warp_dense_fwd(cur, L.in_dim, w_obs[j][l], L.out_dim, cat, out_off, bufs.obs_cat + (int64_t)tr * net.E + out_off, lane);
-        else warp_dense_fwd(cur, L.in_dim, w_obs[j][l], L.out_dim, nxt, 0, bufs.obs_act[j][l] + (int64_t)tr * L.out_dim, lane);
-        float* t = cur; cur = nxt; nxt = t;
-      }
-      in_off += ff.in_dim;
-      out_off += ff.out_dim;
-    }
-    float* cur = cat;
-    float* nxt = va;
-    for (int l = 0; l < net.obs_final.num_layers; ++l) {
-      const ppb_linear_desc& L = net.obs_final.layers[l];
-      const bool last = l == net.obs_final.num_layers - 1;
-      warp_dense_fwd(cur, L.in_dim, w_fin[l], L.out_dim, nxt, 0,
-                     (last ? bufs.obs_emb : bufs.fin_act[l]) + (int64_t)tr * L.out_dim, lane);
-      float* t = cur; cur = nxt; nxt = (t == cat) ? vb : t;
-    }
-    if (bufs.emb_k_hi) {
-      for (int k = lane; k < net.E; k += 32) {
+  const float* xr = act + L.xoff;
+  float* yr = act + L.yoff;
+  float* y = L.y;
+  float* ek_hi = last ? P.emb_k_hi : nullptr;
+  float* ek_lo = P.emb_k_lo;
+  float* em_hi = P.emb_mn_hi;
+  float* em_lo = P.emb_mn_lo;
+  const long long kb = P.emb_kb;
+  for (int n = g; n - (g & 3) < out_dim; n += kRows) {
+    float acc[kMT];
+#pragma unroll
+    for (int t = 0; t < kMT; ++t) acc[t] = 0.f;
+    const float* wr = w + n * pitch;
+    const int kend = n < out_dim ? in_dim : 0;
+    for (int k = s; k < kend; k += kSlices) {
+      const float wv = wr[k];
+#pragma unroll
+      for (int t = 0; t < kMT; ++t) acc[t] = fmaf(wv, xr[t * A + k], acc[t]);
+    }
+#pragma unroll
+    for (int t = 0; t < kMT; ++t) acc[t] = group_sum(acc[t]);
+    if (s < nt && n < out_dim) {
+      const float v = fmaxf(pick(acc, s) + bias[n], 0.f);
+      const int tr = tr0 + s;
+      yr[s * A + n] = v;
+      y[(int64_t)tr * ldy + n] = v;
+      if (ek_hi) {
         float hi, lo;
-        tc::split_tf32(cur[k], hi, lo);
-        const int64_t ok = tc::packed_offset(tr, k, bufs.emb_kb);
-        bufs.emb_k_hi[ok] = hi;
-        if (bufs.emb_k_lo) bufs.emb_k_lo[ok] = lo;
-        if (bufs.emb_mn_hi) {
-          const int64_t om = tc::packed_offset_mn(tr, k, bufs.emb_kb);
-          bufs.emb_mn_hi[om] = hi;
-          if (bufs.emb_mn_lo) bufs.emb_mn_lo[om] = lo;
+        tc::split_tf32(v, hi, lo);
+        const int64_t ok = tc::packed_offset(tr, n, kb);
+        ek_hi[ok] = hi;
+        if (ek_lo) ek_lo[ok] = lo;
+        if (em_hi) {
+          const int64_t om = tc::packed_offset_mn(tr, n, kb);
+          em_hi[om] = hi;
+          if (em_lo) em_lo[om] = lo;
         }
       }
     }
-    __syncwarp();
-  }
-}
-
-__device__ __forceinline__ void warp_dense_dx(const float* dy, int out_dim, const float* w, int in_dim,
-                                              const float* __restrict__ x, float* dx, float* gdx, int lane) {
-  const int pitch = in_dim | 1;
-  const bool p0 = lane < in_dim, p1 = lane + 32 < in_dim, p2 = lane + 64 < in_dim;
-  const float x0 = p0 ? __ldg(x + lane) : 0.f, x1 = p1 ? __ldg(x + lane + 32) : 0.f, x2 = p2 ? __ldg(x + lane + 64) : 0.f;
-  const float* c0 = w + (p0 ? lane : 0);
-  const float* c1 = w + (p1 ? lane + 32 : 0);
-  const float* c2 = w + (p2 ? lane + 64 : 0);
-  float a0 = 0.f, a1 = 0.f, a2 = 0.f;
-  if (in_dim <= 32) {
-#pragma unroll 4
-    for (int n = 0; n < out_dim; ++n) a0 = fmaf(dy[n], c0[n * pitch], a0);
-  } else if (in_dim <= 64) {
-#pragma unroll 4
-    for (int n = 0; n < out_dim; ++n) { const float g = dy[n]; a0 = fmaf(g, c0[n * pitch], a0); a1 = fmaf(g, c1[n * pitch], a1); }
-  } else {
-#pragma unroll 4
-    for (int n = 0; n < out_dim; ++n) { const float g = dy[n]; a0 = fmaf(g, c0[n * pitch], a0); a1 = fmaf(g, c1[n * pitch], a1); a2 = fmaf(g, c2[n * pitch], a2); }
-  }
-  if (p0) { a0 = x0 > 0.f ? a0 : 0.f; dx[lane] = a0; gdx[lane] = a0; }
-  if (p1) { a1 = x1 > 0.f ? a1 : 0.f; dx[lane + 32] = a1; gdx[lane + 32] = a1; }
-  if (p2) { a2 = x2 > 0.f ? a2 : 0.f; dx[lane + 64] = a2; gdx[lane + 64] = a2; }
-  __syncwarp();
-}
-
-__global__ void __launch_bounds__(kWarps * 32) k_bwd2_dx(Net net, const float* __restrict__ arena, int B, int traces_per_cta,
-                                                         Bufs bufs, DBufs dbufs) {
+  }
+}
+
+__global__ void __launch_bounds__(kThreads) k_fwd(const __grid_constant__ Plan P, const float* __restrict__ arena, int B,
+                                                  int traces_per_cta) {
   ppb_pdl_trigger();
-  ppb_pdl_wait();
-  extern __shared__ float smem[];
-  float* p = smem;
-  const float* w_obs[PPB_MAX_OBS][PPB_MAX_FF_LAYERS];
-  const float* w_fin[PPB_MAX_FF_LAYERS];
-  for (int j = 0; j < net.num_obs; ++j)
-    for (int l = 0; l < net.obs_ff[j].num_layers; ++l) {
-      w_obs[j][l] = p;
-      if (l > 0) p = stage_layer(p, arena, net.obs_ff[j].layers[l]);
-    }
-  for (int l = 0; l < net.obs_final.num_layers; ++l) { w_fin[l] = p; p = stage_layer(p, arena, net.obs_final.layers[l]); }
-  const int warp = threadIdx.x >> 5, lane = threadIdx.x & 31, E = net.E;
-  float* va = p + warp * 3 * W2;
-  float* vb = va + W2;
-  float* vc = vb + W2;
-  cp_async_wait_all();
-  __syncthreads();
-  const int t0 = blockIdx.x * traces_per_cta;
-  for (int tr = t0 + warp; tr < t0 + traces_per_cta && tr < B; tr += kWarps) {
-    for (int k = lane; k < E; k += 32) {
-      int64_t o = (int64_t)tr * E + k;
-      float g = bufs.obs_emb[o] > 0.f ? dbufs.d_obs_emb[o] : 0.f;
-      va[k] = g;
-      dbufs.d_obs_emb[o] = g;
-    }
-    __syncwarp();
-    float* cur = va;
-    float* nxt = vb;
-    for (int l = net.obs_final.num_layers - 1; l >= 0; --l) {
-      const ppb_linear_desc& L = net.obs_final.layers[l];
-      const float* x = (l == 0 ? bufs.obs_cat : bufs.fin_act[l - 1]) + (int64_t)tr * L.in_dim;
-      float* gdx = (l == 0 ? dbufs.d_obs_cat : dbufs.d_fin_act[l - 1]) + (int64_t)tr * L.in_dim;
-      warp_dense_dx(cur, L.out_dim, w_fin[l], L.in_dim, x, nxt, gdx, lane);
-      float* t = cur; cur = nxt; nxt = t;
-    }
-    float* dcat = cur;
-    float* scratch = nxt;
-    int out_off = 0;
-    for (int j = 0; j < net.num_obs; ++j) {
-      const ppb_ff_desc& ff = net.obs_ff[j];
-      const float* dy = dcat + out_off;
-      float* o1 = scratch;
-      float* o2 = vc;
-      for (int l = ff.num_layers - 1; l >= 1; --l) {
-        const ppb_linear_desc& L = ff.layers[l];
-        const float* x = bufs.obs_act[j][l - 1] + (int64_t)tr * L.in_dim;
-        warp_dense_dx(dy, L.out_dim, w_obs[j][l], L.in_dim, x, o1, dbufs.d_obs_act[j][l - 1] + (int64_t)tr * L.in_dim, lane);
-        dy = o1;
-        float* t = o1; o1 = o2; o2 = t;
-      }
-      out_off += ff.out_dim;
-    }
-    __syncwarp();
-  }
-}
-
-struct DwLayer { const float* dy; const float* x; int ldy, ldx, out_dim, in_dim, start, pad_; int64_t w_off, b_off; };
-struct DwTable { int n_layers, total; DwLayer layer[PPB_MAX_OBS * PPB_MAX_FF_LAYERS + PPB_MAX_FF_LAYERS]; };
-
-__global__ void __launch_bounds__(256) k_dw(DwTable tab, int B, int b_chunk, float* __restrict__ grad) {
+  extern __shared__ __align__(16) float smem[];
+  const int n_layers = P.n_layers, A = P.A;
+  float* act = smem + P.w_floats;
+  for (int i = 0; i < n_layers; ++i) stage_layer(smem, arena, P.L[i]);
+  const int t_begin = blockIdx.x * traces_per_cta;
+  const int t_end = min(B, t_begin + traces_per_cta);
+  for (int c0 = t_begin; c0 < t_end; c0 += kMT) {
+    const int nt = min(kMT, t_end - c0);
+    for (int i = 0; i < n_layers; ++i) {
+      const Layer& L = P.L[i];
+      if (L.dxoff < 0) load_rows(act + L.xoff, A, L.x, L.ldx, c0, nt, L.in_dim);
+    }
+    cp_async_wait_all();
+    __syncthreads();
+    for (int i = 0; i < n_layers; ++i) {
+      layer_fwd(P, P.L[i], smem, act, c0, nt, i == n_layers - 1);
+      __syncthreads();
+    }
+  }
+}
+
+__device__ __forceinline__ void layer_dx(const Plan& P, const Layer& L, const float* smem, const float* act, float* dz,
+                                         int nt) {
+  const int g = threadIdx.x / kSlices, s = threadIdx.x % kSlices;
+  const int in_dim = L.in_dim, out_dim = L.out_dim, pitch = L.pitch, A = P.A, Dz = P.Dz;
+  const float* w = smem + L.sw;
+  const float* dr = dz + L.dzoff;
+  const float* xr = act + L.xoff;
+  float* dxr = dz + L.dxoff;
+  for (int k = g; k - (g & 3) < in_dim; k += kRows) {
+    float acc[kMT];
+#pragma unroll
+    for (int t = 0; t < kMT; ++t) acc[t] = 0.f;
+    const int nend = k < in_dim ? out_dim : 0;
+    for (int n = s; n < nend; n += kSlices) {
+      const float wv = w[n * pitch + k];
+#pragma unroll
+      for (int t = 0; t < kMT; ++t) acc[t] = fmaf(wv, dr[t * Dz + n], acc[t]);
+    }
+#pragma unroll
+    for (int t = 0; t < kMT; ++t) acc[t] = group_sum(acc[t]);
+    if (s < nt && k < in_dim) dxr[s * Dz + k] = xr[s * A + k] > 0.f ? pick(acc, s) : 0.f;
+  }
+}
+
+__device__ __forceinline__ void layer_partial(const Plan& P, const Layer& L, const float* act, const float* dz, float* part,
+                                              int nt) {
+  const int in_dim = L.in_dim, out_dim = L.out_dim, A = P.A, Dz = P.Dz;
+  const int nw = out_dim * in_dim;
+  const float* dr = dz + L.dzoff;
+  const float* xr = act + L.xoff;
+  float* pr = part + L.part;
+  for (int e = threadIdx.x; e < nw + out_dim; e += kThreads) {
+    float v = 0.f;
+    if (e < nw) {
+      const int n = e / in_dim, k = e - n * in_dim;
+#pragma unroll
+      for (int t = 0; t < kMT; ++t)
+        if (t < nt) v = fmaf(dr[t * Dz + n], xr[t * A + k], v);
+    } else {
+#pragma unroll
+      for (int t = 0; t < kMT; ++t)
+        if (t < nt) v += dr[t * Dz + e - nw];
+    }
+    pr[e] += v;
+  }
+}
+
+__global__ void __launch_bounds__(kThreads) k_bwd(const __grid_constant__ Plan P, const float* __restrict__ arena,
+                                                  const float* __restrict__ d_emb, float* __restrict__ grad, int B,
+                                                  int traces_per_cta) {
   ppb_pdl_trigger();
-  ppb_pdl_wait();
-  __shared__ float part[8][33];
-  const int lane = threadIdx.x & 31, warp = threadIdx.x >> 5;
-  const int idx = blockIdx.x * 32 + lane;
-  float s = 0.f;
-  int li = 0, e = 0, nw = 0;
-  const bool live = idx < tab.total;
-  if (live) {
-    while (li + 1 < tab.n_layers && tab.layer[li + 1].start <= idx) ++li;
-    const DwLayer& L = tab.layer[li];
-    e = idx - L.start;
-    nw = L.out_dim * L.in_dim;
-    const int b0 = blockIdx.y * b_chunk, b1 = min(B, b0 + b_chunk);
-    if (e < nw) {
-      const int n = e / L.in_dim, k = e - n * L.in_dim;
-      const float* dy = L.dy + n;
-      const float* x = L.x + k;
-#pragma unroll 8
-      for (int b = b0 + warp; b < b1; b += 8) s = fmaf(__ldg(dy + (int64_t)b * L.ldy), __ldg(x + (int64_t)b * L.ldx), s);
-    } else {
-      const float* dy = L.dy + (e - nw);
-#pragma unroll 8
-      for (int b = b0 + warp; b < b1; b += 8) s += __ldg(dy + (int64_t)b * L.ldy);
-    }
-  }
-  part[warp][lane] = s;
-  __syncthreads();
-  if (warp == 0 && live) {
-    float t = 0.f;
-#pragma unroll
-    for (int w = 0; w < 8; ++w) t += part[w][lane];
-    const DwLayer& L = tab.layer[li];
-    if (t != 0.f) atomicAdd(grad + (e < nw ? L.w_off + e : L.b_off + (e - nw)), t);
-  }
-}
-
-}
+  extern __shared__ __align__(16) float smem[];
+  const int n_layers = P.n_layers, A = P.A, Dz = P.Dz, E = P.E, part_floats = P.part_floats;
+  float* act = smem + P.w_floats;
+  float* dz = act + kMT * A;
+  float* part = dz + kMT * Dz;
+  for (int i = 0; i < n_layers; ++i)
+    if (P.L[i].dxoff >= 0) stage_layer(smem, arena, P.L[i]);
+  for (int i = threadIdx.x; i < part_floats; i += kThreads) part[i] = 0.f;
+  const int t_begin = blockIdx.x * traces_per_cta;
+  const int t_end = min(B, t_begin + traces_per_cta);
+  const int zoff = P.L[n_layers - 1].dzoff, eoff = P.L[n_layers - 1].yoff;
+  const float* emb = P.L[n_layers - 1].y;
+  bool waited = false;
+  for (int c0 = t_begin; c0 < t_end; c0 += kMT) {
+    const int nt = min(kMT, t_end - c0);
+    for (int i = 0; i < n_layers; ++i) {
+      const Layer& L = P.L[i];
+      load_rows(act + L.xoff, A, L.x, L.ldx, c0, nt, L.in_dim);
+    }
+    load_rows(act + eoff, A, emb, E, c0, nt, E);
+    if (!waited) { ppb_pdl_wait(); waited = true; }
+    load_rows(dz + zoff, Dz, d_emb, E, c0, nt, E);
+    cp_async_wait_all();
+    __syncthreads();
+    for (int idx = threadIdx.x; idx < nt * E; idx += kThreads) {
+      const int t = idx / E, k = idx - t * E;
+      if (!(act[t * A + eoff + k] > 0.f)) dz[t * Dz + zoff + k] = 0.f;
+    }
+    __syncthreads();
+    for (int i = n_layers - 1; i >= 0; --i) {
+      if (P.L[i].dxoff < 0) continue;
+      layer_dx(P, P.L[i], smem, act, dz, nt);
+      __syncthreads();
+    }
+    for (int i = 0; i < n_layers; ++i) layer_partial(P, P.L[i], act, dz, part, nt);
+    __syncthreads();
+  }
+  if (!waited) { ppb_pdl_wait(); cp_async_wait_all(); }
+  tcc::cluster_sync_all();
+  const uint32_t rank = tcc::cluster_ctarank();
+  const uint32_t part_addr = (uint32_t)__cvta_generic_to_shared(part);
+  int li = 0, lpart = P.L[0].part, lnext = n_layers > 1 ? P.L[1].part : part_floats, lnw = P.L[0].out_dim * P.L[0].in_dim;
+  int64_t lw = P.L[0].w_off, lb = P.L[0].b_off;
+  for (int e = rank * kThreads + threadIdx.x; e < part_floats; e += kCluster * kThreads) {
+    float v = 0.f;
+#pragma unroll
+    for (int r = 0; r < kCluster; ++r) v += tcc::ld_cluster(tcc::map_to_rank(part_addr + 4u * (uint32_t)e, (uint32_t)r));
+    while (e >= lnext) {
+      ++li;
+      const Layer& L = P.L[li];
+      lpart = L.part; lnw = L.out_dim * L.in_dim; lw = L.w_off; lb = L.b_off;
+      lnext = li + 1 < n_layers ? P.L[li + 1].part : part_floats;
+    }
+    const int le = e - lpart;
+    if (v != 0.f) atomicAdd(grad + (le < lnw ? lw + le : lb + (le - lnw)), v);
+  }
+  tcc::cluster_sync_all();
+}
+
+}
```

Result: faster. 1.514 million (median of 6 runs) (+3.8%).
